# awslabs/crowd-coachable-recommendations

Hardware: AMD Instinct MI355X
Metric: queries/sec, exhaustive inner-product top-100 retrieval (NQ-shaped 2,681,468 x 768 bf16 corpus) (higher is better)
Workload: dtype bf16

## Files before the change

### crowd-coachable-recommendations_amd/ccrec_amd/_lib.py

```python
import ctypes
import os

_HERE = os.path.dirname(os.path.abspath(__file__))
LIB_PATH = os.path.join(os.path.dirname(_HERE), "lib", "libccr_hip.so")

CCR_OK = 0
CCR_ERR_INVALID, CCR_ERR_HIP, CCR_ERR_WORKSPACE, CCR_ERR_BLOCK_ID = -1, -2, -3, -4
DTYPE_F32, DTYPE_F16, DTYPE_BF16 = 0, 1, 2
SEARCH_DEFAULT, SEARCH_FORCE_DENSE, SEARCH_FORCE_FUSED, SEARCH_ASYNC = 0, 1, 2, 4
SCORES_CANONICAL, SCORES_MFMA = 0, 1

EXPORTS = [
    "ccr_last_error", "ccr_version", "ccr_pack_bf16", "ccr_pack_bf16_ex", "ccr_meanpool_pack_bf16", "ccr_meanpool_pack_bf16_ex", "ccr_index_create",
    "ccr_index_create_with_norms", "ccr_index_destroy",
    "ccr_index_rows", "ccr_index_dim", "ccr_search_workspace_bytes", "ccr_search", "ccr_search_last_stats",
    "ccr_merge_topk", "ccr_merge_topk_strided", "ccr_apply_block", "ccr_inbatch_ce_workspace_bytes", "ccr_inbatch_ce_fwd", "ccr_inbatch_ce_bwd", "ccr_inbatch_ce_bwd_dev", "ccr_rank_metrics",
    "ccr_search_finish", "ccr_scores", "ccr_search_blocked_workspace_bytes", "ccr_search_blocked",
    "ccr_search_sparse_prior_workspace_bytes", "ccr_search_sparse_prior", "ccr_colsum_bf16", "ccr_meanpool_bwd", "ccr_bm25_index_create", "ccr_bm25_index_destroy", "ccr_bm25_search_workspace_bytes",
    "ccr_bm25_search", "ccr_pack_bf16_padded", "ccr_shard_message_bytes", "ccr_search_shard", "ccr_shard_message_fill", "ccr_merge_shard_messages",
    "ccr_attention_bf16", "ccr_add_layernorm", "ccr_meanpool_pack_bf16_packed", "ccr_embed_layernorm", "ccr_gelu_bf16",
    "ccr_attention_half", "ccr_add_layernorm_half", "ccr_embed_layernorm_half", "ccr_gelu_half", "ccr_merge_short_lists",
    "ccr_bm25_search_workspace_bytes_k", "ccr_bm25_search_last_stats", "ccr_bm25_index_set_idf", "ccr_inbatch_pack3_bf16", "ccr_inbatch_ce_fwd_f32",
    "ccr_search_stream_wait_main_pass", "ccr_pool_ce_workspace_bytes", "ccr_pool_ce_fwd", "ccr_pool_ce_fwd_f32", "ccr_pool_ce_bwd_dev",
    "ccr_bpr_sample", "ccr_bpr_frozen_workspace_bytes", "ccr_bpr_frozen_fwd", "ccr_bpr_frozen_bwd_dev",
    "ccr_attention_fwd_train_half", "ccr_attention_bwd_workspace_bytes", "ccr_attention_bwd_half", "ccr_add_layernorm_bwd_half", "ccr_gelu_bwd_half",
    "ccr_dropout_bits_rows", "ccr_dropout_bits_attention", "ccr_dropout_apply", "ccr_attention_fwd_train_drop_half", "ccr_attention_bwd_drop_half",
    "ccr_add_layernorm_drop_half", "ccr_add_layernorm_bwd_drop_half", "ccr_search_last_main_split",
    "ccr_search_last_threshold_phases", "ccr_adamw_step",
    "ccr_embed_layernorm_train_half", "ccr_embed_layernorm_bwd_half", "ccr_embedding_grad", "ccr_meanpool_bwd_packed",
    "ccr_pack_half_ex", "ccr_pack_half_padded", "ccr_meanpool_pack_half_ex", "ccr_meanpool_pack_half_packed", "ccr_index_create_half",
    "ccr_index_create_with_norms_half", "ccr_index_dtype", "ccr_colsum_half",
    "ccr_grad_stats_workspace_bytes", "ccr_grad_stats", "ccr_adamw_control_update", "ccr_adamw_step_scaled",
    "ccr_keep_f32", "ccr_rescore_f32_workspace_bytes", "ccr_rescore_f32",
    "ccr_attention_bias_half",
]

MIN_VERSION = 101
BPR_VERSION = 102
ENCODER_TRAIN_VERSION = 103
ENCODER_DROPOUT_VERSION = 104
QSPLIT_VERSION = 105
THR_PHASES_VERSION = 106
OPTIM_VERSION = 107
ENCODER_PACKED_TRAIN_VERSION = 108
HALF_INDEX_VERSION = 109
AMP_OPTIM_VERSION = 110
RANK_F32_VERSION = 111
ATTENTION_BIAS_VERSION = 112

SHARD_HEADER_BYTES = 32
SHARD_MAGIC = 0x4D524343


class ShardHeader(ctypes.Structure):
    _fields_ = [("magic", ctypes.c_uint32), ("n_flagged", ctypes.c_uint32), ("k_valid", ctypes.c_uint32),
                ("n_covered", ctypes.c_uint32), ("row_offset", ctypes.c_int64), ("n_rows", ctypes.c_int64)]


class SearchStats(ctypes.Structure):
    _fields_ = [("path", ctypes.c_int32), ("n_fallback", ctypes.c_int32), ("sample_tiles", ctypes.c_int32),
                ("ranges", ctypes.c_int32), ("cap", ctypes.c_int32), ("sublists", ctypes.c_int32),
                ("n_candidates", ctypes.c_int64), ("ms_sample", ctypes.c_float), ("ms_threshold", ctypes.c_float),
                ("ms_main", ctypes.c_float), ("ms_select", ctypes.c_float), ("ms_fallback", ctypes.c_float),
                ("ms_total", ctypes.c_float), ("n_retried", ctypes.c_int32), ("n_dense", ctypes.c_int32),
                ("main_launches", ctypes.c_int32), ("opt_rank", ctypes.c_int32), ("main_tile_queries", ctypes.c_int32),
                ("skipped_tiles", ctypes.c_int32), ("tile_cap", ctypes.c_int32)]


class AdamwSegment(ctypes.Structure):
    _fields_ = [("param", ctypes.c_void_p), ("grad", ctypes.c_void_p), ("exp_avg", ctypes.c_void_p), ("exp_avg_sq", ctypes.c_void_p),
                ("shadow", ctypes.c_void_p), ("n", ctypes.c_int64), ("decay", ctypes.c_float), ("step_size", ctypes.c_float),
                ("bc2_sqrt", ctypes.c_float), ("shadow_dtype", ctypes.c_int32)]


class AdamwControl(ctypes.Structure):
    _fields_ = [("coef", ctypes.c_float), ("skip", ctypes.c_int32), ("norm", ctypes.c_float), ("scale", ctypes.c_float),
                ("growth_tracker", ctypes.c_int32), ("skipped_total", ctypes.c_int32), ("reserved", ctypes.c_uint32 * 10)]


CONTROL_WORDS = {name: i for i, (name, _) in enumerate(AdamwControl._fields_[:6])}


class CcrError(RuntimeError):
    pass


_lib = None


def load():
    global _lib
    if _lib is not None:
        return _lib
    if not os.path.isfile(LIB_PATH):
        raise CcrError(f"{LIB_PATH} not built: run `python -c 'import __graft_entry__ as g; g.build()'` "
                       f"(or make -C crowd-coachable-recommendations_amd/csrc)")
    lib = ctypes.CDLL(LIB_PATH)
    lib.ccr_version.restype = ctypes.c_int
    have = int(lib.ccr_version())
    if have < MIN_VERSION:
        raise CcrError(f"{LIB_PATH} is version {have}, this binding needs {MIN_VERSION}: rebuild it "
                       f"(python -c 'import __graft_entry__ as g; g.build()')")
    missing = [name for name in EXPORTS if not hasattr(lib, name)]
    if missing:
        raise CcrError(f"{LIB_PATH} lacks {', '.join(missing)}: rebuild it (python -c 'import __graft_entry__ as g; g.build()')")
    vp, i32, i64, f32, sz = ctypes.c_void_p, ctypes.c_int, ctypes.c_int64, ctypes.c_float, ctypes.c_size_t
    lib.ccr_last_error.restype = ctypes.c_char_p
    lib.ccr_last_error.argtypes = []
    lib.ccr_version.restype = i32
    lib.ccr_pack_bf16.argtypes = [vp, vp, vp, i64, i32, i32, vp]
    lib.ccr_pack_bf16_ex.argtypes = [vp, vp, vp, vp, i64, i32, i32, vp]
    lib.ccr_index_create_with_norms.argtypes = [vp, i64, i32, i64, vp, vp, ctypes.POINTER(vp)]
    lib.ccr_meanpool_pack_bf16.argtypes = [vp, i32, vp, vp, vp, i32, i32, i32, i32, vp]
    lib.ccr_meanpool_pack_bf16_ex.argtypes = [vp, i32, vp, vp, vp, vp, vp, i32, i32, i32, i32, vp]
    lib.ccr_index_create.argtypes = [vp, i64, i32, i64, vp, ctypes.POINTER(vp)]
    lib.ccr_index_destroy.argtypes = [vp]
    lib.ccr_index_rows.argtypes = [vp]
    lib.ccr_index_rows.restype = i64
    lib.ccr_index_dim.argtypes = [vp]
    lib.ccr_search_workspace_bytes.argtypes = [vp, i32, i32]
    lib.ccr_search_workspace_bytes.restype = sz
    lib.ccr_search.argtypes = [vp, vp, i32, i32, vp, vp, vp, sz, i32, vp]
    lib.ccr_search_last_stats.argtypes = [vp, ctypes.POINTER(SearchStats)]
    lib.ccr_merge_topk.argtypes = [vp, vp, i32, i32, i32, vp, vp, vp]
    lib.ccr_merge_topk_strided.argtypes = [vp, vp, i64, i64, i32, i32, i32, vp, vp, vp]
    lib.ccr_apply_block.argtypes = [vp, vp, i32, i32, vp, vp, i64, vp, vp, i32, vp]
    lib.ccr_inbatch_ce_workspace_bytes.argtypes = [i32, i32]
    lib.ccr_inbatch_ce_workspace_bytes.restype = sz
    lib.ccr_inbatch_ce_fwd.argtypes = [vp, vp, vp, i32, i32, f32, vp, vp, vp, sz, vp]
    lib.ccr_inbatch_ce_bwd.argtypes = [vp, vp, vp, vp, i32, i32, f32, f32, vp, vp, vp, vp, sz, vp]
    lib.ccr_inbatch_ce_bwd_dev.argtypes = [vp, vp, vp, vp, i32, i32, f32, vp, vp, vp, vp, vp, sz, vp]
    lib.ccr_inbatch_pack3_bf16.argtypes = [vp, vp, vp, i32, i32, vp, vp]
    lib.ccr_inbatch_ce_fwd_f32.argtypes = [vp, vp, vp, i32, i32, f32, vp, vp, vp, vp, sz, vp]
    lib.ccr_pool_ce_workspace_bytes.argtypes = [i32, i32, i32]
    lib.ccr_pool_ce_workspace_bytes.restype = sz
    lib.ccr_pool_ce_fwd.argtypes = [vp, vp, vp, vp, i32, i32, i32, f32, vp, vp, vp, sz, vp]
    lib.ccr_pool_ce_fwd_f32.argtypes = [vp, vp, vp, vp, i32, i32, i32, f32, vp, vp, vp, vp, sz, vp]
    lib.ccr_pool_ce_bwd_dev.argtypes = [vp, vp, vp, vp, vp, i32, i32, i32, f32, vp, vp, vp, vp, vp, sz, vp]
    lib.ccr_bpr_sample.argtypes = [vp, i32, i32, i64, vp, vp, vp, f32, vp, vp, i32, vp, i32, vp, vp]
    lib.ccr_bpr_frozen_workspace_bytes.argtypes = [i32, i32, i32]
    lib.ccr_bpr_frozen_workspace_bytes.restype = sz
    lib.ccr_bpr_frozen_fwd.argtypes = [vp, i64, i32, vp, vp, f32, vp, vp, vp, vp, i32, i32, vp, vp, sz, vp]
    lib.ccr_bpr_frozen_bwd_dev.argtypes = [vp, i64, i32, vp, vp, f32, vp, vp, vp, vp, i32, i32, vp, vp, vp, vp, vp, sz, vp]
    lib.ccr_rank_metrics.argtypes = [vp, i32, i32, vp, vp, vp, i32, vp, vp, vp]
    lib.ccr_search_finish.argtypes = [vp]
    lib.ccr_search_stream_wait_main_pass.argtypes = [vp, vp]
    lib.ccr_search_last_main_split.argtypes = [vp]
    lib.ccr_search_last_threshold_phases.argtypes = [vp]
    lib.ccr_scores.argtypes = [vp, vp, i32, i32, vp, vp]
    lib.ccr_search_blocked_workspace_bytes.argtypes = [vp, i32, i32, vp]
    lib.ccr_search_blocked_workspace_bytes.restype = sz
    lib.ccr_search_blocked.argtypes = [vp, vp, i32, i32, vp, vp, vp, vp, vp, sz, i32, vp]
    lib.ccr_search_sparse_prior_workspace_bytes.argtypes = [vp, i32, i32, vp]
    lib.ccr_search_sparse_prior_workspace_bytes.restype = sz
    lib.ccr_search_sparse_prior.argtypes = [vp, vp, i32, i32, vp, vp, vp, vp, vp, vp, sz, i32, vp]
    lib.ccr_colsum_bf16.argtypes = [vp, i64, i32, vp, vp]
    lib.ccr_meanpool_bwd.argtypes = [vp, vp, vp, i32, i32, i32, i32, vp]
    lib.ccr_bm25_index_create.argtypes = [vp, vp, vp, vp, i64, i64, ctypes.c_double, ctypes.POINTER(vp)]
    lib.ccr_bm25_index_destroy.argtypes = [vp]
    lib.ccr_bm25_search_workspace_bytes.argtypes = [vp, i32, i32]
    lib.ccr_bm25_search_workspace_bytes.restype = sz
    lib.ccr_bm25_search_workspace_bytes_k.argtypes = [vp, i32, i32, i32]
    lib.ccr_bm25_search_workspace_bytes_k.restype = sz
    lib.ccr_bm25_search_last_stats.argtypes = [vp, vp]
    lib.ccr_bm25_index_set_idf.argtypes = [vp, vp, vp, vp]
    lib.ccr_bm25_search.argtypes = [vp, vp, vp, vp, i32, i32, vp, vp, vp, sz, vp]
    lib.ccr_pack_bf16_padded.argtypes = [vp, i64, i32, vp, i32, vp, vp, i32, vp]
    lib.ccr_attention_bf16.argtypes = [vp, vp, vp, vp, i32, i32, i32, i32, ctypes.c_float, vp]
    lib.ccr_add_layernorm.argtypes = [vp, vp, vp, vp, ctypes.c_float, vp, vp, i64, i32, vp]
    lib.ccr_embed_layernorm.argtypes = [vp, i64, vp, i64, vp, i64, vp, vp, vp, vp, vp, ctypes.c_float, vp, vp, i64, i32, vp]
    lib.ccr_gelu_bf16.argtypes = [vp, vp, i64, vp]
    lib.ccr_attention_half.argtypes = [vp, vp, vp, vp, i32, i32, i32, i32, ctypes.c_float, i32, vp]
    lib.ccr_attention_bias_half.argtypes = [vp, vp, vp, vp, vp, i32, i32, i32, i32, i32, ctypes.c_float, i32, vp]
    lib.ccr_add_layernorm_half.argtypes = [vp, vp, vp, vp, ctypes.c_float, vp, vp, i64, i32, i32, vp]
    lib.ccr_embed_layernorm_half.argtypes = [vp, i64, vp, i64, vp, i64, vp, vp, vp, vp, vp, ctypes.c_float, vp, vp, i64, i32, i32, vp]
    lib.ccr_gelu_half.argtypes = [vp, vp, i64, i32, vp]
    lib.ccr_attention_fwd_train_half.argtypes = [vp, vp, vp, vp, vp, i32, i32, i32, i32, ctypes.c_float, i32, vp]
    lib.ccr_attention_bwd_workspace_bytes.argtypes = [i32, i32, i32]
    lib.ccr_attention_bwd_workspace_bytes.restype = sz
    lib.ccr_attention_bwd_half.argtypes = [vp, vp, vp, vp, vp, vp, vp, i32, i32, i32, i32, ctypes.c_float, i32, vp, sz, vp]
    lib.ccr_add_layernorm_bwd_half.argtypes = [vp, vp, vp, ctypes.c_float, vp, vp, vp, vp, vp, i64, i32, i32, vp, sz, vp]
    lib.ccr_gelu_bwd_half.argtypes = [vp, vp, vp, i64, i32, vp]
    u64, u32, f64 = ctypes.c_uint64, ctypes.c_uint32, ctypes.c_double
    lib.ccr_dropout_bits_rows.argtypes = [vp, i64, i32, u64, u32, f64, vp]
    lib.ccr_dropout_bits_attention.argtypes = [vp, vp, vp, vp, i64, i32, i32, i32, u64, u32, f64, vp]
    lib.ccr_dropout_apply.argtypes = [vp, vp, f32, vp, vp, i64, i32, i32, vp]
    lib.ccr_attention_fwd_train_drop_half.argtypes = [vp, vp, vp, vp, vp, vp, f32, i32, i32, i32, i32, f32, i32, vp]
    lib.ccr_attention_bwd_drop_half.argtypes = [vp, vp, vp, vp, vp, vp, vp, vp, f32, vp, i32, i32, i32, i32, f32, i32, vp, sz, vp]
    lib.ccr_add_layernorm_drop_half.argtypes = [vp, vp, f32, vp, vp, vp, f32, vp, vp, i64, i32, i32, vp]
    lib.ccr_add_layernorm_bwd_drop_half.argtypes = [vp, vp, f32, vp, vp, f32, vp, vp, vp, vp, vp, i64, i32, i32, vp, sz, vp]
    lib.ccr_adamw_step.argtypes = [vp, i32, f32, f32, f32, f32, vp]
    lib.ccr_grad_stats_workspace_bytes.argtypes = [vp, i32]
    lib.ccr_grad_stats_workspace_bytes.restype = i64
    lib.ccr_grad_stats.argtypes = [vp, i32, vp, vp]
    lib.ccr_adamw_control_update.argtypes = [vp, vp, i64, f32, i32, ctypes.c_double, ctypes.c_double, i32, vp, vp, vp]
    lib.ccr_adamw_step_scaled.argtypes = [vp, i32, f32, f32, f32, f32, vp, vp]
    lib.ccr_embed_layernorm_train_half.argtypes = [vp, i64, vp, i64, vp, i64, vp, vp, vp, vp, vp, f32, vp, f32, vp, vp, i64, i32, i32, vp]
    lib.ccr_embed_layernorm_bwd_half.argtypes = [vp, i64, vp, i64, vp, i64, vp, vp, vp, vp, f32, vp, f32, vp, vp, vp, vp, i64, i32, vp, sz, vp]
    lib.ccr_embedding_grad.argtypes = [vp, vp, vp, i64, i32, vp, i64, vp]
    lib.ccr_meanpool_bwd_packed.argtypes = [vp, vp, vp, vp, i32, i32, i32, vp]
    lib.ccr_meanpool_pack_bf16_packed.argtypes = [vp, i32, vp, vp, vp, vp, vp, vp, i32, i32, i32, vp]
    lib.ccr_pack_half_ex.argtypes = [vp, vp, vp, vp, i64, i32, i32, i32, vp, vp]
    lib.ccr_pack_half_padded.argtypes = [vp, i64, i32, vp, i32, vp, vp, i32, i32, vp, vp]
    lib.ccr_meanpool_pack_half_ex.argtypes = [vp, i32, vp, vp, vp, vp, vp, i32, i32, i32, i32, i32, vp, vp]
    lib.ccr_meanpool_pack_half_packed.argtypes = [vp, i32, vp, vp, vp, vp, vp, vp, i32, i32, i32, i32, vp, vp]
    lib.ccr_index_create_half.argtypes = [vp, i64, i32, i32, i64, vp, ctypes.POINTER(vp)]
    lib.ccr_index_create_with_norms_half.argtypes = [vp, i64, i32, i32, i64, vp, vp, ctypes.POINTER(vp)]
    lib.ccr_index_dtype.argtypes = [vp]
    lib.ccr_colsum_half.argtypes = [vp, i64, i32, i32, vp, vp]
    lib.ccr_keep_f32.argtypes = [vp, vp, i32, i32, vp, vp, i64, i32, vp]
    lib.ccr_rescore_f32_workspace_bytes.argtypes = [i32, i32, i32, i32]
    lib.ccr_rescore_f32_workspace_bytes.restype = sz
    lib.ccr_rescore_f32.argtypes = [vp, vp, i64, i32, vp, vp, i32, i32, i32, i64, vp, vp, vp, vp, vp, vp, vp, sz, vp]
    lib.ccr_shard_message_bytes.argtypes = [i32, i32]
    lib.ccr_shard_message_bytes.restype = sz
    lib.ccr_search_shard.argtypes = [vp, vp, i32, i32, vp, vp, sz, i32, vp]
    lib.ccr_shard_message_fill.argtypes = [vp, i32, i32, i32, vp, vp, i64, i64, vp]
    lib.ccr_merge_shard_messages.argtypes = [vp, i64, i32, i32, i32, vp, vp, vp]
    lib.ccr_merge_short_lists.argtypes = [vp, i64, i32, i32, i32, i32, vp, vp, vp, vp, vp]
    for name in EXPORTS:
        fn = getattr(lib, name)
        if fn.restype is ctypes.c_int and name not in ("ccr_version", "ccr_index_dim", "ccr_index_dtype"):
            fn.restype = i32
    _lib = lib
    return lib


def check(rc, what=""):
    if rc != CCR_OK:
        msg = load().ccr_last_error().decode("utf-8", "replace")
        if rc == CCR_ERR_BLOCK_ID:
            raise AssertionError("block id not found")
        raise CcrError(f"{what} failed ({rc}): {msg}")
```

### crowd-coachable-recommendations_amd/csrc/ccr_api.hip

```cpp
#include <stdarg.h>
#include <stdlib.h>
#include <string.h>

#include <math.h>

#include <algorithm>
#include <mutex>
#include <set>
#include <utility>
#include <vector>

#include "ccr_index.h"
#include "ccr_narrow.h"
#include "ccr_topk_device.h"

namespace ccr {

static thread_local char g_err[512] = "";
void set_error(const char *fmt, ...) {
    va_list ap;
    va_start(ap, fmt);
    vsnprintf(g_err, sizeof(g_err), fmt, ap);
    va_end(ap);
}

}

using namespace ccr;

namespace {
constexpr int SLAB_SLOTS = 1024, SLAB_SLOT_BYTES = 256, MAX_DEVICES = 64;
struct Slab {
    char *base = nullptr;
    char *host = nullptr;
    std::vector<int> free_slots;
};
constexpr int SLAB_HOST_BYTES = 64;
std::mutex g_slab_mutex;
Slab g_slabs[MAX_DEVICES];

int slab_take(int device, uint32_t **out, volatile uint32_t **host_out) {
    std::lock_guard<std::mutex> lock(g_slab_mutex);
    CCR_REQUIRE(device >= 0 && device < MAX_DEVICES, "device ordinal %d out of range", device);
    Slab &sl = g_slabs[device];
    if (!sl.base) {
        CCR_HIP_CHECK(hipMalloc((void **)&sl.base, (size_t)SLAB_SLOTS * SLAB_SLOT_BYTES));
        if (hipHostMalloc((void **)&sl.host, (size_t)SLAB_SLOTS * SLAB_HOST_BYTES, hipHostMallocDefault) != hipSuccess) {
            (void)hipFree(sl.base);
            sl.base = nullptr;
            set_error("ccr_index_create: hipHostMalloc of the pinned flag lines failed");
            return CCR_ERR_HIP;
        }
        for (int i = SLAB_SLOTS - 1; i >= 0; --i) sl.free_slots.push_back(i);
    }
    if (sl.free_slots.empty()) {
        set_error("ccr_index_create: more than %d live indices on device %d", SLAB_SLOTS, device);
        return CCR_ERR_INVALID;
    }
    *out = reinterpret_cast<uint32_t *>(sl.base + (size_t)sl.free_slots.back() * SLAB_SLOT_BYTES);
    *host_out = reinterpret_cast<volatile uint32_t *>(sl.host + (size_t)sl.free_slots.back() * SLAB_HOST_BYTES);
    sl.free_slots.pop_back();
    return CCR_OK;
}

void slab_give(int device, uint32_t *p) {
    if (!p || device < 0 || device >= MAX_DEVICES) return;
    std::lock_guard<std::mutex> lock(g_slab_mutex);
    Slab &sl = g_slabs[device];
    sl.free_slots.push_back((int)((reinterpret_cast<char *>(p) - sl.base) / SLAB_SLOT_BYTES));
}
}

extern "C" const char *ccr_last_error(void) { return g_err; }
extern "C" int ccr_version(void) { return 112; }

extern "C" int ccr_index_destroy(ccr_index *ix);

namespace {
struct CachedBlock {
    void *p;
    size_t bytes;
};
std::vector<CachedBlock> g_blocks[MAX_DEVICES];
constexpr size_t BLOCK_CACHE_ENTRIES = 8;

int block_take(int device, size_t bytes, void **out, size_t *got) {
    CCR_REQUIRE(device >= 0 && device < MAX_DEVICES, "device ordinal %d out of range", device);
    bytes = (bytes + 4095) / 4096 * 4096;
    {
        std::lock_guard<std::mutex> lock(g_slab_mutex);
        auto &v = g_blocks[device];
        for (size_t i = 0; i < v.size(); ++i)
            if (v[i].bytes >= bytes && v[i].bytes <= 2 * bytes) {
                *out = v[i].p;
                *got = v[i].bytes;
                v.erase(v.begin() + i);
                return CCR_OK;
            }
    }
    CCR_HIP_CHECK(hipMalloc(out, bytes));
    *got = bytes;
    return CCR_OK;
}

void block_give(int device, void *p, size_t bytes) {
    if (!p) return;
    void *drop = nullptr;
    if (device >= 0 && device < MAX_DEVICES && bytes <= ((size_t)64 << 20)) {
        std::lock_guard<std::mutex> lock(g_slab_mutex);
        auto &v = g_blocks[device];
        v.push_back({p, bytes});
        if (v.size() > BLOCK_CACHE_ENTRIES) {
            drop = v.front().p;
            v.erase(v.begin());
        }
    } else {
        drop = p;
    }
    if (drop) (void)hipFree(drop);
}
}

int ccr::ensure_dynamic_lds(const void *kernel, size_t lds) {
    static std::mutex mu;
    static std::set<std::pair<const void *, int>> done;
    int dev = 0;
    CCR_HIP_CHECK(hipGetDevice(&dev));
    std::lock_guard<std::mutex> lock(mu);
    if (done.count({kernel, dev})) return CCR_OK;
    CCR_HIP_CHECK(hipFuncSetAttribute(kernel, hipFuncAttributeMaxDynamicSharedMemorySize, (int)lds));
    done.insert({kernel, dev});
    return CCR_OK;
}

static int index_create_impl(const uint16_t *D_bf16, int half_dtype, int64_t n_rows, int dim, int64_t global_row_offset, const float *row_bounds,
                             void *stream, ccr_index **out) {
    CCR_REQUIRE(D_bf16 && out, "ccr_index_create: null pointer");
    if (const int rc = check_half("ccr_index_create", half_dtype)) return rc;
    CCR_REQUIRE(n_rows >= 1 && n_rows < ((int64_t)1 << 32), "ccr_index_create: n_rows=%lld out of range [1, 2^32)",
                (long long)n_rows);
    CCR_REQUIRE(dim >= 8 && dim % 8 == 0 && dim <= 4096, "ccr_index_create: dim=%d must be a multiple of 8 in [8, 4096]", dim);
    CCR_REQUIRE((uintptr_t)D_bf16 % 16 == 0, "ccr_index_create: corpus pointer must be 16-byte aligned");
    hipStream_t s = (hipStream_t)stream;
    ccr_index *ix = new ccr_index();
    memset(ix, 0, sizeof(*ix));
    ix->D = D_bf16;
    ix->dtype = half_dtype;
    ix->n_rows = n_rows;
    ix->dim = dim;
    ix->offset = ix->id_out = global_row_offset;
    ix->knobs = read_knobs();
    auto build = [&]() -> int {
        CCR_HIP_CHECK(hipGetDevice(&ix->device));
        CCR_HIP_CHECK(hipDeviceGetAttribute(&ix->num_cu, hipDeviceAttributeMultiprocessorCount, ix->device));
        int rc = slab_take(ix->device, &ix->dmax_bits, &ix->host_flags);
        if (rc != CCR_OK) return rc;
        const int64_t tiles = (n_rows + TILE_DOCS - 1) / TILE_DOCS;
        void *tn = nullptr;
        rc = block_take(ix->device, (size_t)tiles * 4, &tn, &ix->tile_bytes);
        if (rc != CCR_OK) return rc;
        ix->tile_norm = (float *)tn;
        uint32_t *tile_bits = reinterpret_cast<uint32_t *>(ix->tile_norm);
        if (row_bounds) {
            ix->row_norm = row_bounds;
            rc = launch_tile_norms(row_bounds, n_rows, tile_bits, ix->dmax_bits, s);
            if (rc != CCR_OK) return rc;
        } else {
            void *rn = nullptr;
            rc = block_take(ix->device, (size_t)n_rows * 4, &rn, &ix->row_bytes);
            if (rc != CCR_OK) return rc;
            ix->row_norm = ix->row_norm_own = (float *)rn;
            CCR_HIP_CHECK(hipMemsetAsync(ix->dmax_bits, 0, 4, s));
            CCR_HIP_CHECK(hipMemsetAsync(tile_bits, 0, (size_t)tiles * 4, s));
            rc = launch_row_norms(D_bf16, half_dtype, n_rows, dim, ix->row_norm_own, ix->dmax_bits, tile_bits, s);
            if (rc != CCR_OK) return rc;
            CCR_HIP_CHECK(hipStreamSynchronize(s));
        }
        return CCR_OK;
    };
    const int rc = build();
    if (rc != CCR_OK) {
        ccr_index_destroy(ix);
        return rc;
    }
    *out = ix;
    return CCR_OK;
}

extern "C" int ccr_index_create_half(const uint16_t *D, int64_t n_rows, int dim, int half_dtype, int64_t global_row_offset, void *stream,
                                     ccr_index **out) {
    return index_create_impl(D, half_dtype, n_rows, dim, global_row_offset, nullptr, stream, out);
}

extern "C" int ccr_index_create_with_norms_half(const uint16_t *D, int64_t n_rows, int dim, int half_dtype, int64_t global_row_offset,
                                                const float *row_norm_bounds, void *stream, ccr_index **out) {
    CCR_REQUIRE(row_norm_bounds, "ccr_index_create_with_norms: null row_norm_bounds");
    return index_create_impl(D, half_dtype, n_rows, dim, global_row_offset, row_norm_bounds, stream, out);
}

extern "C" int ccr_index_create(const uint16_t *D_bf16, int64_t n_rows, int dim, int64_t global_row_offset, void *stream,
                                ccr_index **out) {
    return ccr_index_create_half(D_bf16, n_rows, dim, CCR_DTYPE_BF16, global_row_offset, stream, out);
}

extern "C" int ccr_index_create_with_norms(const uint16_t *D_bf16, int64_t n_rows, int dim, int64_t global_row_offset,
                                           const float *row_norm_bounds, void *stream, ccr_index **out) {
    return ccr_index_create_with_norms_half(D_bf16, n_rows, dim, CCR_DTYPE_BF16, global_row_offset, row_norm_bounds, stream, out);
}

extern "C" int ccr_index_destroy(ccr_index *ix) {
    if (!ix) return CCR_OK;
    if (ix->pending.active && ix->have_events) (void)hipEventSynchronize(ix->ev[EV_ASYNC_END]);
    ix->pending.active = false;
    slab_give(ix->device, ix->dmax_bits);
    block_give(ix->device, ix->tile_norm, ix->tile_bytes);
    block_give(ix->device, ix->row_norm_own, ix->row_bytes);
    if (ix->have_events)
        for (int i = 0; i < EV_COUNT; ++i)
            if (ix->ev[i]) (void)hipEventDestroy(ix->ev[i]);
    delete ix;
    return CCR_OK;
}

extern "C" int64_t ccr_index_rows(const ccr_index *ix) { return ix ? ix->n_rows : -1; }
extern "C" int ccr_index_dim(const ccr_index *ix) { return ix ? ix->dim : -1; }
extern "C" int ccr_index_dtype(const ccr_index *ix) { return ix ? ix->dtype : -1; }

extern "C" size_t ccr_search_workspace_bytes(const ccr_index *ix, int n_q, int k) {
    if (!ix || n_q <= 0 || k <= 0) return 0;
    Plan a = make_plan(ix->n_rows, ix->dim, n_q, k, CCR_SEARCH_DEFAULT, ix->num_cu, ix->knobs);
    Plan b = make_plan(ix->n_rows, ix->dim, n_q, k, CCR_SEARCH_FORCE_DENSE, ix->num_cu, ix->knobs);
    Plan c = make_plan(ix->n_rows, ix->dim, n_q, k, CCR_SEARCH_FORCE_FUSED, ix->num_cu, ix->knobs);
    return std::max({a.total, b.total, c.total}) + 256;
}

extern "C" int ccr_search_stream_wait_main_pass(const ccr_index *ix, void *stream) {
    CCR_REQUIRE(ix, "ccr_search_stream_wait_main_pass: null index");
    if (!ix->main_pass_recorded) return CCR_OK;
    CCR_HIP_CHECK(hipStreamWaitEvent((hipStream_t)stream, ix->ev[EV_MAIN_END], 0));
    return CCR_OK;
}

extern "C" int ccr_search_last_stats(const ccr_index *ix, ccr_search_stats *stats) {
    CCR_REQUIRE(ix && stats, "ccr_search_last_stats: null pointer");
    CCR_REQUIRE(!ix->pending.active, "ccr_search_last_stats: an asynchronous search is pending (call ccr_search_finish first)");
    *stats = ix->stats;
    return CCR_OK;
}

extern "C" int ccr_search_last_main_split(const ccr_index *ix) {
    if (!ix || ix->plan_nq <= 0 || !ix->plan.fused) return 0;
    return ix->plan.main_qsplit;
}

extern "C" int ccr_search_last_threshold_phases(const ccr_index *ix) {
    if (!ix || ix->plan_nq <= 0 || !ix->plan.fused) return 0;
    return ix->thr_phases_used;
}

static int dense_for_list(const ccr_index *ix, const uint16_t *Q, const uint32_t *d_qlist, int n, int k, float *scratch, int64_t rows_per_chunk,
                          float *out_scores, int64_t *out_ids, hipStream_t s) {
    for (int lo = 0; lo < n; lo += (int)rows_per_chunk) {
        const int m = std::min<int64_t>(rows_per_chunk, n - lo);
        int rc = launch_dense_scores(ix->D, ix->dtype, ix->n_rows, ix->dim, Q, d_qlist ? d_qlist + lo : nullptr, lo, m, nullptr, scratch, s);
        if (rc != CCR_OK) return rc;
        rc = launch_dense_select(scratch, ix->n_rows, k, d_qlist ? d_qlist + lo : nullptr, lo, m, nullptr, ix->id_out, out_scores, out_ids, s);
        if (rc != CCR_OK) return rc;
    }
    return CCR_OK;
}

static bool margin_path_ok(const ccr_index *ix, int k) { return ix->dim % 8 == 0 && k <= MAX_K; }
static int64_t tiles_of(const ccr_index *ix) { return (ix->n_rows + TILE_DOCS - 1) / TILE_DOCS; }

static GemmArgs gemm_args(const ccr_index *ix, const uint16_t *Q, int n_q, int nq_pad) {
    GemmArgs g;
    memset(&g, 0, sizeof(g));
    g.D = ix->D;
    g.n_rows = ix->n_rows;
    g.dim = ix->dim;
    g.Q = Q;
    g.n_q = n_q;
    g.nq_pad = nq_pad;
    g.qblocks = nq_pad / TILE_Q;
    g.item_end = INT32_MAX;
    return g;
}

static GemmArgs filter_args(const ccr_index *ix, const Plan &p, const SearchWs &w, const uint16_t *Q, int n_q, int nq_pad, int qblocks,
                            int qgroups, const float *thr, const float *cq, const CandLayout &lay) {
    GemmArgs g = gemm_args(ix, Q, n_q, nq_pad);
    g.qblocks = qblocks;
    g.qgroups = qgroups;
    g.n_vt = p.tiles;
    g.tile_stride = 1;
    g.ranges = p.ranges;
    g.thr = thr;
    g.cq = cq;
    g.tile_norm = ix->tile_norm;
    g.cnt = w.cnt;
    g.cand = w.cand;
    g.lay = lay;
    return g;
}

static ThresholdArgs threshold_args(const ccr_index *ix, const SearchWs &w) {
    const Plan &p = ix->plan;
    ThresholdArgs t{};
    t.gmax = w.gmax, t.n_groups = (int64_t)p.sample_tiles * GROUPS_PER_TILE, t.sample_stride = p.sample_stride;
    t.n_q = ix->pending.n_q, t.nq_pad = p.nq_pad, t.k = ix->pending.k, t.qnorm = w.qnorm;
    t.dmax_bits = ix->dmax_bits, t.dim = ix->dim, t.tile_norm = ix->tile_norm;
    t.thr = w.thr, t.cq = w.cq, t.phases = ix->knobs.thr_phases;
    return t;
}

static ThresholdUpdateArgs update_args(const ccr_index *ix, const SearchWs &w) {
    ThresholdUpdateArgs u{};
    u.cand = w.cand, u.cnt = w.cnt, u.sp = ix->plan.sublists;
    u.n_q = ix->pending.n_q, u.nq_pad = ix->plan.nq_pad, u.k = ix->pending.k;
    u.cq = w.cq, u.tile_norm = ix->tile_norm, u.thr = w.thr;
    return u;
}

static SelectArgs select_args(const ccr_index *ix, const SearchWs &w) {
    const Plan &p = ix->plan;
    const auto &pd = ix->pending;
    SelectArgs a{};
    a.cand = w.cand, a.cnt = w.cnt, a.n_q = pd.n_q, a.nq_pad = p.nq_pad;
    a.k = pd.k, a.rescore_cap = p.rescore_cap, a.regular_cap = p.rescore_regular, a.compact = p.select_compact;
    a.D = ix->D, a.dt = ix->dtype, a.dim = ix->dim, a.n_rows = ix->n_rows;
    a.tile_norm = ix->tile_norm, a.row_norm = ix->row_norm, a.dmax_bits = ix->dmax_bits, a.id_offset = ix->id_out;
    a.Q = pd.Q, a.thr = w.thr, a.cq = w.cq;
    a.out_scores = pd.out_scores, a.out_ids = pd.out_ids;
    return a;
}

static int store_scores(const ccr_index *ix, const uint16_t *Q, int n_q, int ranges, float *out, int64_t pitch, hipStream_t s) {
    GemmArgs g = gemm_args(ix, Q, n_q, (int)round_up(n_q, TILE_Q));
    g.n_vt = tiles_of(ix);
    g.tile_stride = 1;
    g.ranges = ranges;
    g.qgroups = 1;
    g.store = out;
    g.store_pitch = pitch;
    return launch_gemm(g, ix->dtype, ix->knobs.mfma16 != 0 ? MAIN_16X16 : MAIN_32X32, EPI_STORE, std::max(NUM_XCD, ix->num_cu / NUM_XCD * NUM_XCD), s);
}

static int margin_for_rows(const ccr_index *ix, const uint16_t *Qc, const float *hint, const uint32_t *out_rows, int n, int k, float *scratch,
                           size_t scratch_bytes, float *out_scores, int64_t *out_ids, uint32_t *flag_count, uint32_t *flag_list, hipStream_t s) {
    const int64_t pitch = round_up(ix->n_rows, 4);
    int64_t chunk = (int64_t)(scratch_bytes / ((size_t)pitch * 4));
    CCR_REQUIRE(chunk >= 1, "margin path: no room for one score row");
    if (chunk > TILE_Q) chunk = chunk / TILE_Q * TILE_Q;
    const int ranges = (int)round_up(std::min<int64_t>(std::max<int64_t>(1, tiles_of(ix) / 4), 1024), NUM_XCD);
    for (int lo = 0; lo < n; lo += (int)chunk) {
        const int m = std::min<int64_t>(chunk, n - lo);
        const uint16_t *Q = Qc + (int64_t)lo * ix->dim;
        int rc = store_scores(ix, Q, m, ranges, scratch, pitch, s);
        if (rc != CCR_OK) return rc;
        rc = launch_margin_select(scratch, pitch, ix->n_rows, k, ix->dim, Q, ix->D, ix->dtype, ix->tile_norm, ix->row_norm, ix->dmax_bits,
                                  hint ? hint + lo : nullptr, out_rows ? out_rows + lo : nullptr, lo, m, ix->id_out, out_scores, out_ids, flag_count, flag_list, s);
        if (rc != CCR_OK) return rc;
    }
    return CCR_OK;
}

static int run_main_pass(const ccr_index *ix, const Plan &p, const SearchWs &w, const uint16_t *Q, int n_q, hipStream_t s) {
    GemmArgs gm = filter_args(ix, p, w, Q, n_q, p.nq_pad, p.main_qblocks, p.main_qgroups, w.thr, w.cq, p.cand);
    gm.qsplit = p.main_qsplit;
    if (p.skip_sampled) {
        gm.n_vt = p.tiles - p.sample_tiles;
        gm.skip_stride = (int)p.sample_stride;
        gm.skip_count = p.sample_tiles;
    }
    const int nrc = NUM_XCD / gm.qgroups, qb_per = gm.qblocks / gm.qgroups, items = p.ranges / nrc * qb_per;
    const int bounds[4] = {0, p.item_a, p.item_b, items};
    ThresholdUpdateArgs u = update_args(ix, w);
    u.lay = p.cand, u.qb_per = qb_per, u.tile_q = p.tile_q, u.top = p.item_b ? w.top : nullptr;
    int done = 0;
    for (int ph = 1; ph < 4; ++ph) {
        if (bounds[ph] <= done) continue;
        if (done > 0) {
            const int rl_full = done / qb_per;
            u.part_blocks = done % qb_per;
            u.nsub = rl_full * nrc * p.sublists;
            u.nsub_part = u.part_blocks ? (rl_full + 1) * nrc * p.sublists : 0;
            u.top_out = bounds[ph] < items && ph < 3;
            const int rc = launch_threshold_update(u, s);
            if (rc != CCR_OK) return rc;
            u.prev_nsub = u.nsub, u.prev_part = u.nsub_part, u.prev_blocks = u.part_blocks, u.top_in = true;
        }
        gm.item_begin = done;
        gm.item_end = bounds[ph];
        const MainKernel kind = p.tile_q == WIDE_Q ? MAIN_WIDE : p.mfma16 ? MAIN_16X16 : MAIN_32X32;
        const int rc = launch_gemm(gm, ix->dtype, kind, EPI_FILTER, p.grid, s);
        if (rc != CCR_OK) return rc;
        done = bounds[ph];
    }
    return CCR_OK;
}

static int run_narrow_pass(const ccr_index *ix, const Plan &p, const SearchWs &w, const uint16_t *Q, int n_q, hipStream_t s) {
    NarrowArgs na;
    memset(&na, 0, sizeof(na));
    na.D = ix->D;
    na.n_rows = ix->n_rows;
    na.dim = ix->dim;
    na.Q = Q;
    na.n_q = n_q;
    na.q_stride = narrow_query_stride(ix->dim);
    na.thr = w.thr;
    na.cq = w.cq;
    na.tile_norm = ix->tile_norm;
    na.cand = w.cand;
    na.cnt = w.cnt;
    na.cap = p.first_lay.cap[0];
    na.groups = p.narrow_groups;
    int ngrid = ix->knobs.narrow_grid > 0 ? ix->knobs.narrow_grid : ix->num_cu;
    const int64_t blocks = (ix->n_rows + 16 * NARROW_WAVES - 1) / (16 * NARROW_WAVES);
    if ((int64_t)ngrid > blocks) ngrid = (int)std::max<int64_t>(1, blocks);
    if (p.narrow_groups == 2) ngrid = std::max(16, ngrid / 16 * 16);
    return launch_narrow_filter(na, ix->dtype, p.narrow, ngrid, s);
}

static int read_words(void *host, const void *dev, int n, hipStream_t s) {
    CCR_HIP_CHECK(hipMemcpyAsync(host, dev, (size_t)n * 4, hipMemcpyDeviceToHost, s));
    CCR_HIP_CHECK(hipStreamSynchronize(s));
    return CCR_OK;
}


static int fused_stats(ccr_index *ix, uint32_t nflag, unsigned long long ncand) {
    const Plan &p = ix->plan;
    ccr_search_stats &st = ix->stats;
    float a = 0, b = 0;
    CCR_HIP_CHECK(hipEventElapsedTime(&st.ms_sample, ix->ev[EV_SAMPLE_BEGIN], ix->ev[EV_SAMPLE_END]));
    CCR_HIP_CHECK(hipEventElapsedTime(&a, ix->ev[EV_BEGIN], ix->ev[EV_SAMPLE_BEGIN]));
    CCR_HIP_CHECK(hipEventElapsedTime(&b, ix->ev[EV_SAMPLE_END], ix->ev[EV_MAIN_BEGIN]));
    st.ms_threshold = a + b;
    CCR_HIP_CHECK(hipEventElapsedTime(&st.ms_main, ix->ev[EV_MAIN_BEGIN], ix->ev[EV_MAIN_END]));
    CCR_HIP_CHECK(hipEventElapsedTime(&st.ms_select, ix->ev[EV_MAIN_END], ix->ev[EV_SELECT_END]));
    CCR_HIP_CHECK(hipEventElapsedTime(&st.ms_total, ix->ev[EV_BEGIN], ix->ev[EV_SELECT_END]));
    st.path = 1;
    st.n_fallback = (int32_t)nflag;
    st.sample_tiles = p.sample_tiles;
    st.ranges = p.narrow ? 1 : p.ranges;
    st.cap = p.narrow ? p.first_lay.cap[0] : p.cap;
    st.sublists = p.narrow ? p.first_sp : p.sublists;
    st.main_launches = 1 + (p.item_a ? 1 : 0) + (p.item_b ? 1 : 0);
    st.opt_rank = p.opt_rank;
    st.tile_cap = p.opt_rank ? p.tile_cap : 0;
    st.skipped_tiles = p.skip_sampled ? p.sample_tiles : 0;
    st.main_tile_queries = p.narrow ? 0 : p.tile_q;
    st.n_candidates = (int64_t)ncand;
    return CCR_OK;
}

static int recover_thresholds(const ccr_index *ix, const SearchWs &w, int nflag) {
    hipStream_t s = ix->pending.stream;
    ThresholdArgs t = threshold_args(ix, w);
    t.thr = w.thr_safe, t.cq = w.cq_safe;
    const int rc = launch_threshold(t, s);
    if (rc != CCR_OK) return rc;
    return launch_underfilled_to_retry(w.flag_list, 0, nflag, w.thr_safe, w.thr, s);
}

static int to_dense(const SearchWs &w, const uint32_t *list, int n, int &n_dense, hipStream_t s) {
    CCR_HIP_CHECK(hipMemcpyAsync(w.dense_list + n_dense, list, (size_t)n * 4, hipMemcpyDeviceToDevice, s));
    n_dense += n;
    return CCR_OK;
}

static int retry_group(ccr_index *ix, const SearchWs &w, const uint32_t *cur, int n_cur, int &n_dense) {
    const Plan &p = ix->plan;
    const auto &pd = ix->pending;
    hipStream_t s = pd.stream;
    const int nsub_all = p.ranges * p.sublists;
    for (int round = 0;; ++round) {
        int rc = launch_gather_queries(pd.Q, ix->dim, cur, n_cur, w.thr, w.cq, w.Q2, w.thr2, w.cq2, s);
        if (rc != CCR_OK) return rc;
        const int pad2 = (int)round_up(n_cur, TILE_Q);
        const int64_t cap2 = std::min<int64_t>(8192, (int64_t)(w.cand_bytes / 8) / ((int64_t)nsub_all * pad2) / 4 * 4);
        if (cap2 < 16) break;
        const CandLayout lay2 = one_segment((int)cap2);
        CCR_HIP_CHECK(hipMemsetAsync(w.cnt, 0, (size_t)nsub_all * pad2 * 4, s));
        CCR_HIP_CHECK(hipMemsetAsync(w.flag2, 0, 64, s));
        const GemmArgs g = filter_args(ix, p, w, w.Q2, n_cur, pad2, pad2 / TILE_Q, pick_qgroups(pad2 / TILE_Q, ix->dim, ix->knobs), w.thr2, w.cq2, lay2);
        rc = launch_gemm(g, ix->dtype, p.mfma16 ? MAIN_16X16 : MAIN_32X32, EPI_FILTER, p.grid, s);
        if (rc != CCR_OK) return rc;
        SelectArgs sel = select_args(ix, w);
        sel.ranges = nsub_all, sel.sp = p.sublists, sel.lay = lay2, sel.n_q = n_cur, sel.nq_pad = pad2;
        sel.Q = w.Q2, sel.thr = w.thr2, sel.cq = w.cq2, sel.out_rows = cur;
        sel.flag_count = w.flag2, sel.flag_list = w.flag2 + 16;
        rc = launch_select_rescore(sel, s);
        if (rc != CCR_OK) return rc;
        ix->stats.n_retried += n_cur;
        uint32_t again = 0;
        rc = read_words(&again, w.flag2, 1, s);
        if (rc != CCR_OK || again == 0) return rc;
        uint32_t *next = (cur == w.list_b) ? w.list_c : w.list_b;
        rc = launch_partition_flags(w.flag2 + 16, 0, (int)again, next, w.dense_list + n_dense, w.counts, s);
        if (rc != CCR_OK) return rc;
        uint32_t hc[2] = {0, 0};
        rc = read_words(hc, w.counts, 2, s);
        if (rc != CCR_OK) return rc;
        n_dense += (int)hc[1];
        const uint32_t *list = cur;
        const int n = n_cur;
        cur = next;
        n_cur = (int)hc[0];
        if (n_cur == 0 || round == 2 || n_cur >= n) break;
        ThresholdUpdateArgs u = update_args(ix, w);
        u.nsub = nsub_all, u.lay = lay2, u.n_q = n, u.nq_pad = pad2, u.cq = w.cq2, u.thr = w.thr2;
        rc = launch_threshold_update(u, s);
        if (rc != CCR_OK) return rc;
        rc = launch_scatter_thresholds(list, n, w.thr2, w.thr, s);
        if (rc != CCR_OK) return rc;
    }
    return n_cur > 0 ? to_dense(w, cur, n_cur, n_dense, s) : CCR_OK;
}

static int retry_flagged(ccr_index *ix, const SearchWs &w, int n_retry, int &n_dense) {
    const Plan &p = ix->plan;
    const auto &pd = ix->pending;
    const int nsub_all = p.ranges * p.sublists;
    if (nsub_all > 2048) return to_dense(w, w.retry_list, n_retry, n_dense, pd.stream);
    ThresholdUpdateArgs u = update_args(ix, w);
    u.nsub = p.first_nsub, u.sp = p.first_sp, u.lay = p.first_lay;
    int rc = launch_threshold_update(u, pd.stream);
    if (rc != CCR_OK) return rc;
    const int64_t want_cap = std::min<int64_t>(8192, 4 * (int64_t)p.cap);
    int64_t group = (int64_t)(w.cand_bytes / 8) / ((int64_t)nsub_all * want_cap) / TILE_Q * TILE_Q;
    group = std::max<int64_t>(TILE_Q, std::min<int64_t>(group, round_up(n_retry, TILE_Q)));
    for (int g0 = 0; g0 < n_retry && rc == CCR_OK; g0 += (int)group)
        rc = retry_group(ix, w, w.retry_list + g0, std::min<int>((int)group, n_retry - g0), n_dense);
    return rc;
}

static int complete_dense(ccr_index *ix, const SearchWs &w, int n_dense) {
    const Plan &p = ix->plan;
    const auto &pd = ix->pending;
    hipStream_t s = pd.stream;
    const bool margin_in_cand = w.cand_bytes > w.dense_bytes;
    const int64_t fit = (int64_t)(w.cand_bytes / ((size_t)ix->n_rows * 4)) / 64 * 64;
    const bool fp64_in_cand = n_dense > p.dense_rows_per_chunk && fit >= 64;
    const int64_t chunk = fp64_in_cand ? std::min<int64_t>(fit, 256) : p.dense_rows_per_chunk;
    float *fp64_scr = fp64_in_cand ? (float *)w.cand : w.dense;
    if (!margin_path_ok(ix, pd.k))
        return dense_for_list(ix, pd.Q, w.dense_list, n_dense, pd.k, fp64_scr, chunk, pd.out_scores, pd.out_ids, s);
    CCR_HIP_CHECK(hipMemsetAsync(w.flag2, 0, 64, s));
    for (int lo = 0; lo < n_dense; lo += p.nq_pad) {
        const int m = std::min(p.nq_pad, n_dense - lo);
        int rc = launch_gather_queries(pd.Q, ix->dim, w.dense_list + lo, m, w.thr, w.cq, w.Q2, w.thr2, w.cq2, s);
        if (rc != CCR_OK) return rc;
        rc = margin_for_rows(ix, w.Q2, w.thr2, w.dense_list + lo, m, pd.k, margin_in_cand ? (float *)w.cand : w.dense,
                             margin_in_cand ? w.cand_bytes : w.dense_bytes, pd.out_scores, pd.out_ids, w.flag2, w.flag2 + 16, s);
        if (rc != CCR_OK) return rc;
    }
    uint32_t left = 0;
    const int rc = read_words(&left, w.flag2, 1, s);
    if (rc != CCR_OK || left == 0) return rc;
    return dense_for_list(ix, pd.Q, w.flag2 + 16, (int)left, pd.k, fp64_scr, chunk, pd.out_scores, pd.out_ids, s);
}

static int search_complete(ccr_index *ix) {
    auto &pd = ix->pending;
    hipStream_t s = pd.stream;
    const bool was_async = pd.active;
    pd.active = false;
    const SearchWs w = search_ws(ix->plan, ix->n_rows, ix->dim, pd.n_q, pd.k, pd.ws);
    struct { uint32_t nflag, pad; unsigned long long ncand; } host;
    int rc = CCR_OK;
    if (was_async) {
        CCR_HIP_CHECK(hipEventSynchronize(ix->ev[EV_ASYNC_END]));
        host.nflag = ix->host_flags[0];
        host.ncand = *reinterpret_cast<volatile unsigned long long *>(ix->host_flags + 2);
    } else {
        rc = read_words(&host, w.flag_count, 4, s);
        if (rc != CCR_OK) return rc;
    }
    rc = fused_stats(ix, host.nflag, host.ncand);
    if (rc != CCR_OK || host.nflag == 0) return rc;
    rc = ix->plan.opt_rank ? recover_thresholds(ix, w, (int)host.nflag) : CCR_OK;
    if (rc != CCR_OK) return rc;
    rc = launch_partition_flags(w.flag_list, 0, (int)host.nflag, w.retry_list, w.dense_list, w.counts, s);
    if (rc != CCR_OK) return rc;
    uint32_t hc[2] = {0, 0};
    rc = read_words(hc, w.counts, 2, s);
    if (rc != CCR_OK) return rc;
    int n_dense = (int)hc[1];
    if (hc[0] > 0) rc = retry_flagged(ix, w, (int)hc[0], n_dense);
    if (rc == CCR_OK && n_dense > 0) rc = complete_dense(ix, w, n_dense);
    if (rc != CCR_OK) return rc;
    ix->stats.n_dense += n_dense;
    CCR_HIP_CHECK(hipEventRecord(ix->ev[EV_DONE], s));
    CCR_HIP_CHECK(hipStreamSynchronize(s));
    CCR_HIP_CHECK(hipEventElapsedTime(&ix->stats.ms_fallback, ix->ev[EV_SELECT_END], ix->ev[EV_DONE]));
    ix->stats.ms_total += ix->stats.ms_fallback;
    return CCR_OK;
}

extern "C" int ccr_search_finish(ccr_index *ix) {
    CCR_REQUIRE(ix, "ccr_search_finish: null index");
    return ix->pending.active ? search_complete(ix) : CCR_OK;
}

static int search_dense(ccr_index *ix, const SearchWs &w, const uint16_t *Q, int n_q, int k, float *out_scores, int64_t *out_ids,
                        int flags, hipStream_t s) {
    const bool async = (flags & CCR_SEARCH_ASYNC) != 0;
    const int64_t chunk = ix->plan.dense_rows_per_chunk;
    int rc;
    if (!async && !(flags & CCR_SEARCH_FORCE_DENSE) && margin_path_ok(ix, k)) {
        CCR_HIP_CHECK(hipMemsetAsync(w.flag_count, 0, 64, s));
        rc = margin_for_rows(ix, Q, nullptr, nullptr, n_q, k, w.dense, w.dense_bytes, out_scores, out_ids, w.flag_count, w.flag_list, s);
        if (rc != CCR_OK) return rc;
        uint32_t nf = 0;
        rc = read_words(&nf, w.flag_count, 1, s);
        if (rc != CCR_OK) return rc;
        ix->stats.n_fallback = ix->stats.n_dense = (int32_t)nf;
        if (nf > 0) rc = dense_for_list(ix, Q, w.flag_list, (int)nf, k, w.dense, chunk, out_scores, out_ids, s);
    } else {
        rc = dense_for_list(ix, Q, nullptr, n_q, k, w.dense, chunk, out_scores, out_ids, s);
    }
    if (rc != CCR_OK) return rc;
    CCR_HIP_CHECK(hipEventRecord(ix->ev[EV_DONE], s));
    if (async) return CCR_OK;
    CCR_HIP_CHECK(hipStreamSynchronize(s));
    CCR_HIP_CHECK(hipEventElapsedTime(&ix->stats.ms_total, ix->ev[EV_BEGIN], ix->ev[EV_DONE]));
    ix->stats.ms_fallback = ix->stats.ms_total;
    return CCR_OK;
}

static int search_impl(ccr_index *ix, const uint16_t *Q_bf16, int n_q, int k, float *out_scores, int64_t *out_ids, int64_t id_out,
                       uint32_t *flagged_out, void *workspace, size_t ws_bytes, int flags, void *stream) {
    CCR_REQUIRE(ix && Q_bf16 && out_scores && out_ids, "ccr_search: null pointer");
    CCR_REQUIRE(n_q >= 0, "ccr_search: n_q=%d", n_q);
    CCR_REQUIRE(k >= 1 && k <= MAX_K && (int64_t)k <= ix->n_rows, "ccr_search: k=%d must be in [1, min(n_rows=%lld, %d)]", k,
                (long long)ix->n_rows, MAX_K);
    CCR_REQUIRE((uintptr_t)Q_bf16 % 16 == 0, "ccr_search: query pointer must be 16-byte aligned");
    CCR_REQUIRE(!ix->pending.active, "ccr_search: an asynchronous search is pending on this index (call ccr_search_finish first)");
    memset(&ix->stats, 0, sizeof(ix->stats));
    ix->main_pass_recorded = false;
    ix->thr_phases_used = 0;
    if (n_q == 0) return CCR_OK;
    hipStream_t s = (hipStream_t)stream;
    ix->id_out = id_out;
    const bool async = (flags & CCR_SEARCH_ASYNC) != 0;
    const int plan_flags = flags & ~CCR_SEARCH_ASYNC;
    if (!(ix->plan_nq == n_q && ix->plan_k == k && ix->plan_flags == plan_flags)) {
        ix->plan = make_plan(ix->n_rows, ix->dim, n_q, k, plan_flags, ix->num_cu, ix->knobs);
        ix->plan_nq = n_q;
        ix->plan_k = k;
        ix->plan_flags = plan_flags;
    }
    const Plan p = ix->plan;
    if (!workspace || ws_bytes < p.total || (uintptr_t)workspace % 256 != 0) {
        set_error("ccr_search: workspace %zu bytes (256-byte aligned) required, got %zu at %p", p.total, ws_bytes, workspace);
        return CCR_ERR_WORKSPACE;
    }
    const SearchWs w = search_ws(p, ix->n_rows, ix->dim, n_q, k, (char *)workspace);

    if (!ix->have_events) {
        for (int i = 0; i < EV_COUNT; ++i) CCR_HIP_CHECK(hipEventCreate(&ix->ev[i]));
        ix->have_events = true;
    }
    CCR_HIP_CHECK(hipEventRecord(ix->ev[EV_BEGIN], s));
    if (!p.fused) return search_dense(ix, w, Q_bf16, n_q, k, out_scores, out_ids, flags, s);
    ix->pending = {false, Q_bf16, n_q, k, out_scores, out_ids, (char *)workspace, s};

    CCR_HIP_CHECK(hipMemsetAsync(w.flag_count, 0, 64, s));
    if ((int64_t)p.ranges > p.tiles - (p.skip_sampled ? p.sample_tiles : 0)) CCR_HIP_CHECK(hipMemsetAsync(w.cnt, 0, (size_t)p.ranges * p.nq_pad * p.sublists * 4, s));
    int rc = launch_row_norms(Q_bf16, ix->dtype, n_q, ix->dim, w.qnorm, nullptr, nullptr, s);
    if (rc != CCR_OK) return rc;

    GemmArgs gs = gemm_args(ix, Q_bf16, n_q, p.nq_pad);
    gs.qgroups = p.qgroups;
    gs.n_vt = p.sample_tiles;
    gs.tile_stride = p.sample_stride;
    gs.ranges = p.sample_ranges;
    gs.gmax = w.gmax;
    CCR_HIP_CHECK(hipEventRecord(ix->ev[EV_SAMPLE_BEGIN], s));
    rc = launch_gemm(gs, ix->dtype, MAIN_32X32, EPI_GMAX, p.grid, s);
    if (rc != CCR_OK) return rc;
    CCR_HIP_CHECK(hipEventRecord(ix->ev[EV_SAMPLE_END], s));
    const bool skip_list = p.skip_sampled && ix->knobs.skip_list;
    ThresholdArgs t = threshold_args(ix, w);
    if (p.opt_rank) t.k = p.opt_rank, t.tile_cap = p.tile_cap;
    if (p.narrow) t.zero_cnt = w.cnt, t.zero_per_query = NARROW_SUBLISTS;
    if (skip_list) t.glist = w.glist, t.list_cap = skip_list_cap(p.opt_rank);
    rc = launch_threshold(t, s, &ix->thr_phases_used);
    if (rc != CCR_OK) return rc;

    CCR_HIP_CHECK(hipEventRecord(ix->ev[EV_MAIN_BEGIN], s));
    rc = p.narrow ? run_narrow_pass(ix, p, w, Q_bf16, n_q, s) : run_main_pass(ix, p, w, Q_bf16, n_q, s);
    if (rc != CCR_OK) return rc;
    CCR_HIP_CHECK(hipEventRecord(ix->ev[EV_MAIN_END], s));
    ix->main_pass_recorded = true;
    SelectArgs sel = select_args(ix, w);
    sel.ranges = p.first_nsub, sel.sp = p.first_sp, sel.lay = p.first_lay;
    sel.flag_count = w.flag_count, sel.flag_list = w.flag_list, sel.stat_cand = w.stat_cand;
    if (p.skip_sampled)
        sel.gmax = w.gmax, sel.sample_tiles = p.sample_tiles, sel.sample_stride = (int)p.sample_stride, sel.gmax_pitch = p.nq_pad;
    if (skip_list) sel.glist = w.glist, sel.list_cap = t.list_cap;
    rc = launch_select_rescore(sel, s);
    if (rc != CCR_OK) return rc;
    CCR_HIP_CHECK(hipEventRecord(ix->ev[EV_SELECT_END], s));

    if (!async) return search_complete(ix);
    if (flagged_out) CCR_HIP_CHECK(hipMemcpyAsync(flagged_out, w.flag_count, 4, hipMemcpyDeviceToDevice, s));
    CCR_HIP_CHECK(hipMemcpyAsync((void *)ix->host_flags, w.flag_count, 16, hipMemcpyDeviceToHost, s));
    CCR_HIP_CHECK(hipEventRecord(ix->ev[EV_ASYNC_END], s));
    ix->pending.active = true;
    return CCR_OK;
}

extern "C" int ccr_search(ccr_index *ix, const uint16_t *Q_bf16, int n_q, int k, float *out_scores, int64_t *out_ids,
                          void *workspace, size_t ws_bytes, int flags, void *stream) {
    CCR_REQUIRE(ix, "ccr_search: null index");
    return search_impl(ix, Q_bf16, n_q, k, out_scores, out_ids, ix->offset, nullptr, workspace, ws_bytes, flags, stream);
}

static inline size_t shard_rows_at(int n_q, int k) { return (sizeof(ccr_shard_header) + (size_t)n_q * k * 4 + 15) / 16 * 16; }

extern "C" size_t ccr_shard_message_bytes(int n_q, int k) {
    if (n_q < 0 || k < 1) return 0;
    return (shard_rows_at(n_q, k) + (size_t)n_q * k * 4 + 15) / 16 * 16;
}

extern "C" int ccr_search_shard(ccr_index *ix, const uint16_t *Q_bf16, int n_q, int k, void *message, void *workspace, size_t ws_bytes,
                                int flags, void *stream) {
    CCR_REQUIRE(ix && message, "ccr_search_shard: null pointer");
    CCR_REQUIRE((uintptr_t)message % 16 == 0, "ccr_search_shard: message must be 16-byte aligned");
    CCR_REQUIRE(n_q >= 0 && k >= 1, "ccr_search_shard: bad shape n_q=%d k=%d", n_q, k);
    hipStream_t s = (hipStream_t)stream;
    ccr_shard_header h;
    memset(&h, 0, sizeof(h));
    h.magic = CCR_SHARD_MAGIC;
    h.k_valid = (uint32_t)k;
    h.n_covered = 0u;
    h.row_offset = ix->offset;
    h.n_rows = ix->n_rows;
    int rc = launch_shard_header(h, message, s);
    if (rc != CCR_OK) return rc;
    if (n_q == 0) return CCR_OK;
    char *m = (char *)message;
    uint32_t *flagged = reinterpret_cast<uint32_t *>(m + offsetof(ccr_shard_header, n_flagged));
    return search_impl(ix, Q_bf16, n_q, k, reinterpret_cast<float *>(m + sizeof(ccr_shard_header)),
                       reinterpret_cast<int64_t *>(m + shard_rows_at(n_q, k)), ID_LOCAL_U32, flagged, workspace, ws_bytes, flags, stream);
}

extern "C" int ccr_scores(const ccr_index *ix, const uint16_t *Q_bf16, int n_q, int mode, float *out, void *stream) {
    CCR_REQUIRE(ix && Q_bf16 && out && n_q > 0, "ccr_scores: bad argument");
    CCR_REQUIRE((uintptr_t)Q_bf16 % 16 == 0, "ccr_scores: query pointer must be 16-byte aligned");
    if (mode == CCR_SCORES_CANONICAL)
        return launch_dense_scores(ix->D, ix->dtype, ix->n_rows, ix->dim, Q_bf16, nullptr, 0, n_q, nullptr, out, (hipStream_t)stream);
    CCR_REQUIRE(mode == CCR_SCORES_MFMA, "ccr_scores: unknown mode %d", mode);
    CCR_REQUIRE(ix->dim % 8 == 0, "ccr_scores: CCR_SCORES_MFMA needs dim %% 8 == 0 (dim=%d)", ix->dim);
    return store_scores(ix, Q_bf16, n_q, (int)round_up(std::min<int64_t>(64, tiles_of(ix)), NUM_XCD), out, 0, (hipStream_t)stream);
}
```

### crowd-coachable-recommendations_amd/csrc/ccr_common.h

```cpp
#pragma once
#include <hip/hip_runtime.h>
#include <stdint.h>
#include <stdio.h>

#include <type_traits>

#include "ccr_retrieval.h"

namespace ccr {

void set_error(const char *fmt, ...);

#define CCR_HIP_CHECK(expr)                                                                   \
    do {                                                                                      \
        hipError_t _e = (expr);                                                               \
        if (_e != hipSuccess) {                                                               \
            ccr::set_error("%s failed: %s (%s:%d)", #expr, hipGetErrorString(_e), __FILE__, __LINE__); \
            return CCR_ERR_HIP;                                                               \
        }                                                                                     \
    } while (0)

#define CCR_REQUIRE(cond, ...)            \
    do {                                  \
        if (!(cond)) {                    \
            ccr::set_error(__VA_ARGS__);  \
            return CCR_ERR_INVALID;       \
        }                                 \
    } while (0)

#define CCR_LAUNCH_CHECK()                                                              \
    do {                                                                                \
        hipError_t _e = hipGetLastError();                                              \
        if (_e != hipSuccess) {                                                         \
            ccr::set_error("kernel launch failed: %s (%s:%d)", hipGetErrorString(_e), __FILE__, __LINE__); \
            return CCR_ERR_HIP;                                                         \
        }                                                                               \
    } while (0)

constexpr int TILE_DOCS = 256;
constexpr int TILE_Q = 256;
constexpr int WIDE_Q = 384;
constexpr int TILE_K = 32;
constexpr int GEMM_THREADS = 512;
constexpr int GROUPS_PER_TILE = 16;
constexpr int MAX_K = 4096;
constexpr uint32_t FLAG_DENSE = 0x80000000u;
constexpr int NUM_XCD = 8;

struct CandLayout {
    int nseg;
    int seg_end[3];
    int cap[3];
    long long base[3];
};
__host__ __device__ __forceinline__ void cand_segment(const CandLayout &L, int r, int &cap, int &r0, long long &base) {
    const int g = (r >= L.seg_end[0] ? 1 : 0) + (r >= L.seg_end[1] ? 1 : 0);
    r0 = g ? L.seg_end[g - 1] : 0;
    cap = L.cap[g];
    base = L.base[g];
}
__host__ __device__ __forceinline__ long long cand_sublist(const CandLayout &L, int r, int q, int s, int nq_pad, int sp, int &cap) {
    const int g = (r >= L.seg_end[0] ? 1 : 0) + (r >= L.seg_end[1] ? 1 : 0);
    const int r0 = g ? L.seg_end[g - 1] : 0;
    cap = L.cap[g];
    return L.base[g] + (((long long)(r - r0) * nq_pad + q) * sp) * (long long)cap + s;
}

__host__ __device__ __forceinline__ int64_t unsampled_tile(int64_t v, int s, int n) {
    if (s == 0) return v;
    const uint32_t u = (uint32_t)v, d = (uint32_t)(s - 1);
    return u < (uint32_t)n * d ? (int64_t)(u + u / d + 1u) : v + n;
}

__host__ __device__ __forceinline__ int64_t main_item(int i, int xcd, int qblocks, int qgroups, int qsplit, int ranges, int64_t n_vt, int &r,
                                                      int &qb) {
    const int groups = qsplit ? qsplit : qgroups, g = xcd % groups, rc = xcd / groups, nrc = NUM_XCD / groups;
    const int base = qblocks / groups;
    int rl, b;
    if (qsplit == 0) {
        rl = i / base;
        b = g * base + i % base;
    } else {
        const int rem = qblocks - base * groups;
        const int period = i / qblocks, o = i - period * qblocks;
        int row = g, k = o - g * base;
        if (k < 0) {
            row = o / base;
            k = o - row * base;
        } else if (k >= base + rem) {
            row = (o - rem) / base;
            k = o - rem - row * base;
        }
        rl = period * groups + row;
        b = k >= base ? groups * base + (k - base) : g * base + k;
    }
    const int ri = rc + nrc * rl;
    const int64_t ntile = (n_vt - ri + ranges - 1) / ranges;
    r = ri;
    qb = b;
    return ntile;
}

enum { EPI_FILTER = 0, EPI_GMAX = 1, EPI_STORE = 2 };

struct GemmArgs {
    const uint16_t *D;
    int64_t n_rows;
    int dim;
    const uint16_t *Q;
    int n_q;
    int nq_pad;
    int qblocks;
    int64_t n_vt;
    int64_t tile_stride;
    int ranges;
    int skip_stride, skip_count;
    int qgroups;
    int qsplit;
    int item_begin, item_end;
    const float *thr;
    const float *cq;
    const float *tile_norm;
    uint2 *cand;
    uint32_t *cnt;
    CandLayout lay;
    float *gmax;
    float *store;
    int64_t store_pitch;
};


template <class F>
inline int dispatch_half(int half_dtype, F &&f) {
    return half_dtype == CCR_DTYPE_F16 ? f(std::integral_constant<int, CCR_DTYPE_F16>{}) : f(std::integral_constant<int, CCR_DTYPE_BF16>{});
}
inline int check_half(const char *who, int half_dtype) {
    CCR_REQUIRE(half_dtype == CCR_DTYPE_BF16 || half_dtype == CCR_DTYPE_F16, "%s: half_dtype=%d (CCR_DTYPE_F16 or CCR_DTYPE_BF16)", who, half_dtype);
    return CCR_OK;
}

template <int DT>
__device__ __forceinline__ float elem_to_f32(uint16_t h) {
    if constexpr (DT == CCR_DTYPE_F16)
        return (float)__builtin_bit_cast(_Float16, h);
    else
        return __uint_as_float(((uint32_t)h) << 16);
}
template <int DT>
__device__ __forceinline__ float elem_lo(uint32_t w) {
    if constexpr (DT == CCR_DTYPE_F16)
        return elem_to_f32<DT>((uint16_t)w);
    else
        return __uint_as_float(w << 16);
}
template <int DT>
__device__ __forceinline__ float elem_hi(uint32_t w) {
    if constexpr (DT == CCR_DTYPE_F16)
        return elem_to_f32<DT>((uint16_t)(w >> 16));
    else
        return __uint_as_float(w & 0xffff0000u);
}

__device__ __forceinline__ double wave_sumsq(const float *__restrict__ x, int dim, int lane) {
    double p = 0.0;
    const int nchunk = dim >> 2;
    for (int c = lane; c < nchunk; c += 64) {
        float4 v = reinterpret_cast<const float4 *>(x)[c];
        p = p + (double)v.x * (double)v.x;
        p = p + (double)v.y * (double)v.y;
        p = p + (double)v.z * (double)v.z;
        p = p + (double)v.w * (double)v.w;
    }
#pragma unroll
    for (int off = 32; off >= 1; off >>= 1) p = p + __shfl_xor(p, off, 64);
    return p;
}

__device__ __forceinline__ uint32_t f32_orderable(float f) {
    uint32_t u = __float_as_uint(f);
    return (u & 0x80000000u) ? ~u : (u | 0x80000000u);
}
__device__ __forceinline__ float orderable_to_f32(uint32_t u) {
    return __uint_as_float((u & 0x80000000u) ? (u & 0x7fffffffu) : ~u);
}

constexpr int64_t ID_LOCAL_U32 = INT64_MIN;
__device__ __forceinline__ void store_id(int64_t *out_ids, int64_t pos, int64_t id_offset, uint32_t row) {
    if (id_offset == ID_LOCAL_U32)
        reinterpret_cast<uint32_t *>(out_ids)[pos] = row;
    else
        out_ids[pos] = id_offset + (int64_t)row;
}

__host__ __device__ __forceinline__ float mfma_gamma(int dim) { return (float)dim * 1.1920929e-7f * 1.02f; }

}
```

### crowd-coachable-recommendations_amd/csrc/ccr_index.h

```cpp
#pragma once
#include "ccr_common.h"
#include "ccr_plan.h"

namespace ccr {

enum MainKernel { MAIN_32X32, MAIN_16X16, MAIN_WIDE };
int launch_gemm(const GemmArgs &a, int dt, MainKernel kind, int epi, int grid, hipStream_t s);
int launch_shard_header(const ccr_shard_header &h, void *message, hipStream_t s);
int ensure_dynamic_lds(const void *kernel, size_t lds);
int launch_row_norms(const uint16_t *X, int dt, int64_t rows, int dim, float *norms, uint32_t *max_bits, uint32_t *tile_bits,
                     hipStream_t s);
int launch_tile_norms(const float *row_bounds, int64_t rows, uint32_t *tile_bits, uint32_t *max_bits, hipStream_t s);

struct ThresholdArgs {
    const float *gmax;
    int64_t n_groups, sample_stride;
    int n_q, nq_pad, dim;
    int k;
    int tile_cap = GROUPS_PER_TILE;
    const float *qnorm, *tile_norm;
    const uint32_t *dmax_bits;
    float *thr, *cq;
    uint32_t *zero_cnt = nullptr; int zero_per_query = 0;
    uint32_t *glist = nullptr; int list_cap = 0;
    int phases = 0;
};
int launch_threshold(const ThresholdArgs &a, hipStream_t s, int *phases_used = nullptr);

struct ThresholdUpdateArgs {
    const uint2 *cand;
    const uint32_t *cnt;
    CandLayout lay;
    int sp;
    int n_q, nq_pad, k, nsub;
    const float *cq, *tile_norm;
    float *thr;
    int nsub_part = 0, part_blocks = 0, prev_nsub = 0, prev_part = 0, prev_blocks = 0;
    int qb_per = 1;
    uint32_t *top = nullptr;
    bool top_in = false, top_out = false;
    int tile_q = TILE_Q;
};
int launch_threshold_update(const ThresholdUpdateArgs &a, hipStream_t s);

int select_compact_entries(int dim, int ranges, int rescore_cap, int64_t want);
struct SelectArgs {
    const uint2 *cand;
    const uint32_t *cnt;
    CandLayout lay;
    int ranges, sp, n_q, nq_pad;
    int k, rescore_cap, compact;
    int regular_cap;
    const uint16_t *D;
    int dt, dim;
    int64_t n_rows, id_offset;
    const float *tile_norm, *row_norm;
    const uint32_t *dmax_bits;
    const uint16_t *Q;
    float *thr;
    const float *cq;
    float *out_scores;
    int64_t *out_ids;
    const uint32_t *out_rows = nullptr;
    uint32_t *flag_count, *flag_list;
    unsigned long long *stat_cand = nullptr;
    const float *gmax = nullptr; int sample_tiles = 0, sample_stride = 0, gmax_pitch = 0;
    const uint32_t *glist = nullptr; int list_cap = 0;
};
int launch_select_rescore(const SelectArgs &a, hipStream_t s);
int launch_partition_flags(const uint32_t *flags, int begin, int n, uint32_t *retry_list, uint32_t *dense_list, uint32_t *counts,
                           hipStream_t s);
int launch_underfilled_to_retry(uint32_t *flags, int begin, int n, const float *thr_safe, float *thr, hipStream_t s);
int launch_scatter_thresholds(const uint32_t *list, int n, const float *thr2, float *thr, hipStream_t s);
int launch_gather_queries(const uint16_t *Q, int dim, const uint32_t *list, int n, const float *thr, const float *cq, uint16_t *Q2,
                          float *thr2, float *cq2, hipStream_t s);
int launch_dense_scores(const uint16_t *D, int dt, int64_t n_rows, int dim, const uint16_t *Q, const uint32_t *qlist,
                        int q_begin, int nq_chunk, const uint32_t *count_dev, float *out, hipStream_t s);
int launch_dense_select(const float *scores, int64_t n_rows, int k, const uint32_t *out_rows, int q_begin, int nq_chunk,
                        const uint32_t *count_dev, int64_t id_offset, float *out_scores, int64_t *out_ids, hipStream_t s,
                        bool aggregate = true, const uint32_t *in_rows = nullptr, bool in_rows_compact = false);

int launch_margin_select(const float *scores, int64_t pitch, int64_t n_rows, int k, int dim, const uint16_t *Q, const uint16_t *D, int dt,
                         const float *tile_norm, const float *row_norm, const uint32_t *dmax_bits, const float *hint, const uint32_t *out_rows,
                         int q_begin, int nq_chunk, int64_t id_offset, float *out_scores, int64_t *out_ids, uint32_t *flag_count, uint32_t *flag_list,
                         hipStream_t s);

enum SearchEvent { EV_BEGIN, EV_SAMPLE_BEGIN, EV_SAMPLE_END, EV_MAIN_BEGIN, EV_MAIN_END, EV_SELECT_END, EV_DONE, EV_ASYNC_END, EV_COUNT };

}

struct ccr_index {
    const uint16_t *D;
    int dtype;
    int64_t n_rows;
    int dim;
    int64_t offset;
    int64_t id_out;
    uint32_t *dmax_bits;
    float *tile_norm;
    size_t tile_bytes;
    const float *row_norm;
    float *row_norm_own;
    size_t row_bytes;
    bool have_events;
    int thr_phases_used;
    bool main_pass_recorded;
    int num_cu;
    int device;
    ccr::Knobs knobs;
    hipEvent_t ev[ccr::EV_COUNT];
    volatile uint32_t *host_flags;
    ccr::Plan plan;
    int plan_nq, plan_k, plan_flags;
    ccr_search_stats stats;
    struct {
        bool active;
        const uint16_t *Q;
        int n_q, k;
        float *out_scores;
        int64_t *out_ids;
        char *ws;
        hipStream_t stream;
    } pending;
};
```

### crowd-coachable-recommendations_amd/csrc/ccr_main_pass.hip

```cpp
#include "ccr_gemm_common.h"
#include "ccr_index.h"

namespace ccr {

__device__ __attribute__((aligned(16))) uint32_t g_zero_chunk[4];

__device__ __forceinline__ float load_uniform_f32(const float *p) {
    float v;
    asm volatile("s_load_dword %0, %1, 0x0\n\ts_waitcnt lgkmcnt(0)" : "=s"(v) : "s"(p) : "memory");
    return v;
}

template <int N>
__device__ __forceinline__ void wait_vm() {
    asm volatile("s_waitcnt vmcnt(%0)" ::"n"(N) : "memory");
}

typedef float f32x4v __attribute__((ext_vector_type(4)));

__device__ __forceinline__ float max4_asm(const f32x4v &c) {
    float m;
    asm("v_max3_f32 %0, %1, %2, %3\n\tv_max_f32 %0, %0, %4" : "=&v"(m) : "v"(c[0]), "v"(c[1]), "v"(c[2]), "v"(c[3]));
    return m;
}
__device__ __forceinline__ float max3_asm(float a, float b, float c) {
    float m;
    asm("v_max3_f32 %0, %1, %2, %3" : "=v"(m) : "v"(a), "v"(b), "v"(c));
    return m;
}

__device__ __forceinline__ int64_t real_tile(const GemmArgs &a, int64_t vt) {
    return a.skip_stride ? unsampled_tile(vt, a.skip_stride, a.skip_count) : vt * a.tile_stride;
}

struct ItemWalk {
    int jx, step, xcd, end;
    __device__ __forceinline__ explicit ItemWalk(const GemmArgs &a) {
        xcd = blockIdx.x & (NUM_XCD - 1);
        jx = blockIdx.x >> 3;
        step = gridDim.x >> 3;
        const int count_x = (a.ranges / NUM_XCD) * a.qblocks;
        end = a.item_end < count_x ? a.item_end : count_x;
    }
    __device__ __forceinline__ int first(const GemmArgs &a) const { return a.item_begin + jx; }
    __device__ __forceinline__ int64_t item(const GemmArgs &a, int i, int &r, int &qb) const {
        return main_item(i, xcd, a.qblocks, a.qgroups, a.qsplit, a.ranges, a.n_vt, r, qb);
    }
};


template <int ET>
struct Mfma32 {
    typedef f32x16 Acc;
    static constexpr int TILE = 32, REGS = 16, DT = 4, QT = 2, SUBLISTS = 4;
    struct Frags { bf16x8 a[2][4], b[2][2]; };

    static __device__ __forceinline__ int src_swizzle(int row) { return (row >> 2) & 3; }

    int a_base, b_base, cofs[2];
    __device__ __forceinline__ Mfma32(int lane, int wd, int wq) {
        const int swz = (lane >> 2) & 3;
#pragma unroll
        for (int ks = 0; ks < 2; ++ks) cofs[ks] = (((2 * ks + (lane >> 5)) ^ swz) << 4);
        a_base = (wd * 128 + (lane & 31)) * 64;
        b_base = SUB_Q_REGION + (wq * 64 + (lane & 31)) * 64;
    }
    __device__ __forceinline__ void read(const char *buf, Frags &f) const {
#pragma unroll
        for (int ks = 0; ks < 2; ++ks) {
#pragma unroll
            for (int dt = 0; dt < 4; ++dt) f.a[ks][dt] = *reinterpret_cast<const bf16x8 *>(buf + a_base + dt * 2048 + cofs[ks]);
#pragma unroll
            for (int qt = 0; qt < 2; ++qt) f.b[ks][qt] = *reinterpret_cast<const bf16x8 *>(buf + b_base + qt * 2048 + cofs[ks]);
        }
    }
    static __device__ __forceinline__ void mma(Acc (&acc)[4][2], const Frags &f, bool first) {
        if (first) {
            const f32x16 z = {0.f, 0.f, 0.f, 0.f, 0.f, 0.f, 0.f, 0.f, 0.f, 0.f, 0.f, 0.f, 0.f, 0.f, 0.f, 0.f};
#pragma unroll
            for (int dt = 0; dt < 4; ++dt)
#pragma unroll
                for (int qt = 0; qt < 2; ++qt) acc[dt][qt] = mfma_32x32x16<ET>(f.a[0][dt], f.b[0][qt], z);
        } else {
#pragma unroll
            for (int dt = 0; dt < 4; ++dt)
#pragma unroll
                for (int qt = 0; qt < 2; ++qt) acc[dt][qt] = mfma_32x32x16<ET>(f.a[0][dt], f.b[0][qt], acc[dt][qt]);
        }
#pragma unroll
        for (int dt = 0; dt < 4; ++dt)
#pragma unroll
            for (int qt = 0; qt < 2; ++qt) acc[dt][qt] = mfma_32x32x16<ET>(f.a[1][dt], f.b[1][qt], acc[dt][qt]);
    }

    static __device__ __forceinline__ void tile_max(const Acc (&acc)[4][2], int qt, float (&sub)[4][4], float (&mdt)[4]) {
#pragma unroll
        for (int dt = 0; dt < 4; ++dt) {
#pragma unroll
            for (int g = 0; g < 4; ++g)
                sub[dt][g] = fmaxf(fmaxf(acc[dt][qt][4 * g], acc[dt][qt][4 * g + 1]), fmaxf(acc[dt][qt][4 * g + 2], acc[dt][qt][4 * g + 3]));
            mdt[dt] = fmaxf(fmaxf(sub[dt][0], sub[dt][1]), fmaxf(sub[dt][2], sub[dt][3]));
        }
    }
    static __device__ __forceinline__ void gmax(const Acc (&acc)[4][2], const GemmArgs &a, int64_t vt, int q0, int wd, int wq, int lane) {
        const int h = lane >> 5;
#pragma unroll
        for (int qt = 0; qt < 2; ++qt) {
            float sub[4][4], mdt[4];
            tile_max(acc, qt, sub, mdt);
            const int ql = wq * 64 + qt * 32 + (lane & 31);
#pragma unroll
            for (int dt = 0; dt < 4; ++dt) a.gmax[(vt * GROUPS_PER_TILE + wd * 8 + dt * 2 + h) * a.nq_pad + q0 + ql] = mdt[dt];
        }
    }
    static __device__ __forceinline__ void filter(const Acc (&acc)[4][2], const float (&thr)[2], const float (&cqv)[2], float nt,
                                                  int64_t row_base, const GemmArgs &a, uint2 *const (&clist)[2], uint32_t (&ncand)[2],
                                                  int cap) {
        const uint32_t row32 = (uint32_t)row_base;
        const int64_t left = a.n_rows - row_base;
        const uint32_t rows_left = left <= 0 ? 0u : (left > 128 ? 128u : (uint32_t)left);
#pragma unroll
        for (int qt = 0; qt < 2; ++qt) {
            float sub[4][4], mdt[4];
            tile_max(acc, qt, sub, mdt);
            const float t = fmaf(-cqv[qt], nt, thr[qt]);
            const float mall = fmaxf(fmaxf(mdt[0], mdt[1]), fmaxf(mdt[2], mdt[3]));
            if (__ballot(mall >= t) == 0ull) continue;
#pragma unroll
            for (int dt = 0; dt < 4; ++dt) {
                if (__ballot(mdt[dt] >= t) == 0ull) continue;
#pragma unroll
                for (int g = 0; g < 4; ++g) {
                    if (sub[dt][g] >= t) {
#pragma unroll
                        for (int e2 = 0; e2 < 4; ++e2) {
                            const float v = acc[dt][qt][4 * g + e2];
                            const uint32_t off = (uint32_t)(dt * 32 + 8 * g + e2);
                            if (v >= t && off < rows_left) {
                                if (ncand[qt] < (uint32_t)cap) clist[qt][ncand[qt] * 4] = make_uint2(__float_as_uint(v), row32 + off);
                                ++ncand[qt];
                            }
                        }
                    }
                }
            }
        }
    }
};

template <int ET>
struct Mfma16 {
    typedef f32x4v Acc;
    static constexpr int TILE = 16, REGS = 4, DT = 8, QT = 4, SUBLISTS = 8;
    struct Frags { bf16x8 a[8], b[4]; };

    static __device__ __forceinline__ int src_swizzle(int row) { return ((row >> 2) & 1) << 1; }

    int a_base, b_base;
    __device__ __forceinline__ Mfma16(int lane, int wd, int wq) {
        const int cofs = (((lane >> 4) ^ (((lane >> 2) & 1) << 1)) << 4);
        a_base = (wd * 128 + (lane & 15)) * 64 + cofs;
        b_base = SUB_Q_REGION + (wq * 64 + (lane & 15)) * 64 + cofs;
    }
    __device__ __forceinline__ void read(const char *buf, Frags &f) const {
#pragma unroll
        for (int dt = 0; dt < 8; ++dt) f.a[dt] = *reinterpret_cast<const bf16x8 *>(buf + a_base + dt * 1024);
#pragma unroll
        for (int qt = 0; qt < 4; ++qt) f.b[qt] = *reinterpret_cast<const bf16x8 *>(buf + b_base + qt * 1024);
    }
    static __device__ __forceinline__ void mma(Acc (&acc)[8][4], const Frags &f, bool first) {
        if (first) {
            const f32x4v z = {0.f, 0.f, 0.f, 0.f};
#pragma unroll
            for (int dt = 0; dt < 8; ++dt)
#pragma unroll
                for (int qt = 0; qt < 4; ++qt) acc[dt][qt] = mfma_16x16x32<ET>(f.a[dt], f.b[qt], z);
            return;
        }
#pragma unroll
        for (int dt = 0; dt < 8; ++dt)
#pragma unroll
            for (int qt = 0; qt < 4; ++qt) acc[dt][qt] = mfma_16x16x32<ET>(f.a[dt], f.b[qt], acc[dt][qt]);
    }

    static __device__ __forceinline__ void filter(const Acc (&acc)[8][4], const float (&thr)[4], const float (&cqv)[4], float nt,
                                                  int64_t row_base, const GemmArgs &a, uint2 *const (&clist)[4], uint32_t (&ncand)[4],
                                                  int cap) {
#pragma unroll
        for (int qt = 0; qt < 4; ++qt) {
            float sub[8];
#pragma unroll
            for (int dt = 0; dt < 8; ++dt) sub[dt] = max4_asm(acc[dt][qt]);
            const float t = fmaf(-cqv[qt], nt, thr[qt]);
            float mall = max3_asm(sub[0], sub[1], sub[2]);
            mall = max3_asm(mall, sub[3], sub[4]);
            mall = max3_asm(mall, sub[5], sub[6]);
            mall = fmaxf(mall, sub[7]);
            if (__ballot(mall >= t) == 0ull) continue;
#pragma unroll
            for (int dt = 0; dt < 8; ++dt) {
                if (sub[dt] >= t) {
#pragma unroll
                    for (int e = 0; e < 4; ++e) {
                        const float v = acc[dt][qt][e];
                        const int64_t doc = row_base + dt * 16 + e;
                        if (v >= t && doc < a.n_rows) {
                            if (ncand[qt] < (uint32_t)cap) clist[qt][ncand[qt] * 8] = make_uint2(__float_as_uint(v), (uint32_t)doc);
                            ++ncand[qt];
                        }
                    }
                }
            }
        }
    }
};

template <class S, int EPI, bool TAIL>
__device__ __forceinline__ void main_pass_256(const GemmArgs &a) {
    static_assert(EPI != EPI_GMAX || S::TILE == 32, "EPI_GMAX exists on the 32x32 shape only");
    extern __shared__ __attribute__((aligned(16))) char smem[];

    const int tid = threadIdx.x & (GEMM_THREADS - 1);
    const int lane = tid & 63;
    const int wv = __builtin_amdgcn_readfirstlane(tid >> 6);
    const int wd = wv >> 2;
    const int wq = wv & 3;
    const int lc = lane & (S::TILE - 1);
    const int lh = lane / S::TILE;
    const int cell = wd * (S::SUBLISTS / 2) + lh;
    const bool g1 = (wv >= 4);
    const int KS2 = TAIL ? (a.dim + SUB_K - 1) / SUB_K : a.dim / SUB_K;

    const int srow = wv * 16 + (lane >> 2);
    const int schunk = (lane & 3) ^ S::src_swizzle(srow);
    const S mfma(lane, wd, wq);

    const ItemWalk walk(a);
    for (int item = walk.first(a); item < walk.end; item += walk.step) {
        int r, qb;
        const int64_t ntile = walk.item(a, item, r, qb);
        if (ntile <= 0) continue;
        const int q0 = qb * TILE_Q;

        float thr[S::QT] = {}, cqv[S::QT] = {};
        uint32_t ncand[S::QT] = {};
        uint2 *clist[S::QT] = {};
        int cap = 0;
        if (EPI == EPI_FILTER) {
            int seg_r0;
            long long seg_base;
            cand_segment(a.lay, r, cap, seg_r0, seg_base);
#pragma unroll
            for (int qt = 0; qt < S::QT; ++qt) {
                const int q = q0 + wq * 64 + qt * S::TILE + lc;
                thr[qt] = (q < a.n_q) ? a.thr[q] : __builtin_nanf("");
                cqv[qt] = (q < a.n_q) ? a.cq[q] : 0.f;
                clist[qt] = a.cand + seg_base + ((int64_t)(r - seg_r0) * a.nq_pad + q) * S::SUBLISTS * cap + cell;
            }
#pragma unroll
            for (int qt = 0; qt < S::QT; ++qt) asm volatile("" : "+v"(thr[qt]), "+v"(cqv[qt]));
        }
        float *dst[S::QT] = {};
        if (EPI == EPI_STORE) {
            const int64_t pitch = a.store_pitch ? a.store_pitch : a.n_rows;
#pragma unroll
            for (int qt = 0; qt < S::QT; ++qt) {
                const int q = q0 + wq * 64 + qt * S::TILE + lc;
                if (q < a.n_q) dst[qt] = a.store + (int64_t)q * pitch;
            }
        }
        const uint16_t *qsrc[2];
#pragma unroll
        for (int i = 0; i < 2; ++i) {
            int qrow = q0 + i * 128 + srow;
            if (qrow > a.n_q - 1) qrow = a.n_q - 1;
            qsrc[i] = a.Q + (int64_t)qrow * a.dim + schunk * 8;
        }

        typename S::Acc acc[S::DT][S::QT];
        const int64_t U = ntile * KS2;

        int64_t iu = 0, it = 0;
        int iks = 0;
        const uint16_t *dsrc[2];
        auto tile_ptrs = [&]() {
            const int64_t row0 = real_tile(a, r + it * a.ranges) * TILE_DOCS;
#pragma unroll
            for (int i = 0; i < 2; ++i) {
                int64_t drow = row0 + (i * 128 + srow);
                if (drow > a.n_rows - 1) drow = a.n_rows - 1;
                dsrc[i] = a.D + drow * a.dim + schunk * 8;
            }
        };
        tile_ptrs();
        auto issue = [&]() {
            char *buf = smem + (int)(iu & (RING - 1)) * SUB_BYTES;
            const int k0 = iks * SUB_K;
            if (TAIL && iks == KS2 - 1) {
                const bool in = k0 + schunk * 8 < a.dim;
#pragma unroll
                for (int i = 0; i < 2; ++i)
                    glds16(in ? (const void *)(dsrc[i] + k0) : (const void *)g_zero_chunk, buf + (i * 512 + wv * 64) * 16);
#pragma unroll
                for (int i = 0; i < 2; ++i)
                    glds16(in ? (const void *)(qsrc[i] + k0) : (const void *)g_zero_chunk, buf + SUB_Q_REGION + (i * 512 + wv * 64) * 16);
            } else {
#pragma unroll
                for (int i = 0; i < 2; ++i) glds16(dsrc[i] + k0, buf + (i * 512 + wv * 64) * 16);
#pragma unroll
                for (int i = 0; i < 2; ++i) glds16(qsrc[i] + k0, buf + SUB_Q_REGION + (i * 512 + wv * 64) * 16);
            }
            ++iu;
            if (++iks == KS2) {
                iks = 0;
                ++it;
                tile_ptrs();
            }
        };

        auto epilogue = [&](int64_t vt, int64_t rt, float nt) {
            const int64_t row_base = rt * TILE_DOCS + wd * 128 + 4 * lh;
            if constexpr (EPI == EPI_GMAX) {
                S::gmax(acc, a, vt, q0, wd, wq, lane);
            } else if constexpr (EPI == EPI_FILTER) {
                S::filter(acc, thr, cqv, nt, row_base, a, clist, ncand, cap);
            } else {
                const int64_t pitch = a.store_pitch ? a.store_pitch : a.n_rows;
#pragma unroll
                for (int qt = 0; qt < S::QT; ++qt) {
                    if (!dst[qt]) continue;
#pragma unroll
                    for (int dt = 0; dt < S::DT; ++dt)
#pragma unroll
                        for (int g = 0; g < S::REGS / 4; ++g) {
                            const int64_t doc = row_base + dt * S::TILE + 8 * g;
                            if ((pitch & 3) == 0 && doc + 3 < a.n_rows) {
                                *reinterpret_cast<float4 *>(dst[qt] + doc) = make_float4(acc[dt][qt][4 * g], acc[dt][qt][4 * g + 1],
                                                                                             acc[dt][qt][4 * g + 2], acc[dt][qt][4 * g + 3]);
                            } else {
#pragma unroll
                                for (int e2 = 0; e2 < 4; ++e2)
                                    if (doc + e2 < a.n_rows) dst[qt][doc + e2] = acc[dt][qt][4 * g + e2];
                            }
                        }
                }
            }
        };

        const int npro = U < 3 ? (int)U : 3;
        for (int i = 0; i < npro; ++i) issue();
        if (npro == 3)
            CCR_WAIT_VM(8);
        else if (npro == 2)
            CCR_WAIT_VM(4);
        else
            CCR_WAIT_VM(0);
        CCR_BARRIER();
        if (g1) CCR_BARRIER();

        int cks = 0;
        int64_t ct = 0;
        bool pending = false;
        int64_t pending_vt = 0, pending_rt = 0;
        float pending_nt = 0.f;
        for (int64_t u = 0; u < U; ++u) {
            if (pending) {
                epilogue(pending_vt, pending_rt, pending_nt);
                pending = false;
            }
            if (u + 1 < U) {
                if (u + 2 < U)
                    CCR_WAIT_VM(4);
                else
                    CCR_WAIT_VM(0);
            }
            typename S::Frags f;
            mfma.read(smem + (int)(u & (RING - 1)) * SUB_BYTES, f);
            if (u + 3 < U) issue();
            CCR_WAIT_LGKM0();
            CCR_BARRIER();
            S::mma(acc, f, cks == 0);
            if (++cks == KS2) {
                cks = 0;
                const int64_t vt_done = r + ct * a.ranges;
                const int64_t rt_done = real_tile(a, vt_done);
                const float nt_done = EPI == EPI_FILTER ? load_uniform_f32(a.tile_norm + rt_done) : 0.f;
                if (g1) {
                    epilogue(vt_done, rt_done, nt_done);
                } else {
                    pending = true;
                    pending_vt = vt_done;
                    pending_rt = rt_done;
                    pending_nt = nt_done;
                }
                ++ct;
            }
            CCR_BARRIER();
        }
        if (pending) epilogue(pending_vt, pending_rt, pending_nt);
        if (!g1) CCR_BARRIER();

        if (EPI == EPI_FILTER) {
#pragma unroll
            for (int qt = 0; qt < S::QT; ++qt)
                a.cnt[((int64_t)r * a.nq_pad + q0 + wq * 64 + qt * S::TILE + lc) * S::SUBLISTS + cell] = ncand[qt];
        }
        __syncthreads();
    }
}

template <int ET, int EPI, bool TAIL = false>
__global__ __launch_bounds__(GEMM_THREADS, 2) void gemm_topk_kernel(const GemmArgs a) { main_pass_256<Mfma32<ET>, EPI, TAIL>(a); }
template <int ET, int EPI, bool TAIL = false>
__global__ __launch_bounds__(GEMM_THREADS, 2) void gemm_topk16_kernel(const GemmArgs a) { main_pass_256<Mfma16<ET>, EPI, TAIL>(a); }


__device__ __forceinline__ int fresh_lane() {
    int l;
    asm volatile("v_mbcnt_lo_u32_b32 %0, -1, 0\n\tv_mbcnt_hi_u32_b32 %0, -1, %0" : "=v"(l));
    return l;
}
__device__ __forceinline__ uint32_t lds_offset(const void *p) {
    return (uint32_t)(uintptr_t)(const __attribute__((address_space(3))) void *)p;
}
template <int OFF>
__device__ __forceinline__ uint64_t lds_issue_read_b64(uint32_t addr) {
    uint64_t v;
    asm volatile("ds_read_b64 %0, %1 offset:%2" : "=v"(v) : "v"(addr), "n"(OFF) : "memory");
    return v;
}
template <int OFF>
__device__ __forceinline__ uint32_t lds_issue_read_b32(uint32_t addr) {
    uint32_t v;
    asm volatile("ds_read_b32 %0, %1 offset:%2" : "=v"(v) : "v"(addr), "n"(OFF) : "memory");
    return v;
}
template <int OFF>
__device__ __forceinline__ void lds_issue_write_b32(uint32_t addr, uint32_t v) {
    asm volatile("ds_write_b32 %0, %1 offset:%2" ::"v"(addr), "v"(v), "n"(OFF) : "memory");
}
__device__ __forceinline__ void lds_wait_cells(uint64_t (&tc)[6], uint32_t (&cn)[6]) {
    asm volatile("s_waitcnt lgkmcnt(0)"
                 : "+v"(tc[0]), "+v"(tc[1]), "+v"(tc[2]), "+v"(tc[3]), "+v"(tc[4]), "+v"(tc[5]), "+v"(cn[0]), "+v"(cn[1]), "+v"(cn[2]), "+v"(cn[3]),
                   "+v"(cn[4]), "+v"(cn[5])
                 :
                 : "memory");
}
constexpr int WIDE_SUB_BYTES = (TILE_DOCS + WIDE_Q) * SUB_K * 2;
constexpr int WIDE_Q_REGION = TILE_DOCS * SUB_K * 2;
constexpr int WIDE_RING = 3;
constexpr int WIDE_PIECES = 5;
constexpr int WIDE_QT = 6;
constexpr int WIDE_RING_BYTES = WIDE_RING * WIDE_SUB_BYTES;
constexpr size_t WIDE_LDS = (size_t)WIDE_RING_BYTES + WIDE_Q * 8 + (size_t)(GEMM_THREADS / 64) * WIDE_QT * 64 * 4;

template <int ET>
__global__ __launch_bounds__(GEMM_THREADS, 2) void gemm_topk16w_kernel(const GemmArgs a) {
    extern __shared__ __attribute__((aligned(16))) char smem[];
    float2 *s_tc = reinterpret_cast<float2 *>(smem + WIDE_RING_BYTES);
    uint32_t *s_cnt = reinterpret_cast<uint32_t *>(smem + WIDE_RING_BYTES + WIDE_Q * 8);
    const int wv = __builtin_amdgcn_readfirstlane((int)threadIdx.x >> 6);
    const int wd = wv >> 2;
    const int wq = wv & 3;
    const bool g1 = (wv >= 4);
    const int KS2 = a.dim / SUB_K;
    const uint32_t pitch = (uint32_t)a.dim * 2u;
    uint32_t lane_src, lane_lds;
    {
        const int ln = fresh_lane();
        const int pr = ln >> 2;
        lane_src = (uint32_t)pr * pitch + (uint32_t)(((ln & 3) ^ (((pr >> 2) & 1) << 1)) << 4);
        lane_lds = (uint32_t)((ln & 15) * 64 + (((ln >> 4) ^ (((ln >> 2) & 1) << 1)) << 4));
    }

    const ItemWalk walk(a);
    for (int item = walk.first(a); item < walk.end; item += walk.step) {
        int r, qb;
        const int64_t ntile = walk.item(a, item, r, qb);
        if (ntile <= 0) continue;
        const int q0 = qb * WIDE_Q;

        int cap, seg_r0;
        long long seg_base;
        cand_segment(a.lay, r, cap, seg_r0, seg_base);
        {
            const int ln = fresh_lane();
            const int tid = wv * 64 + ln;
            if (tid < WIDE_Q) {
                const int q = q0 + tid;
                s_tc[tid] = make_float2((q < a.n_q) ? a.thr[q] : __builtin_nanf(""), (q < a.n_q) ? a.cq[q] : 0.f);
            }
#pragma unroll
            for (int qt = 0; qt < WIDE_QT; ++qt) s_cnt[(wv * WIDE_QT + qt) * 64 + ln] = 0u;
        }
        CCR_WAIT_VM(0);

        const int qlimit = (a.n_q - 1 - q0 < WIDE_Q - 1) ? a.n_q - 1 - q0 : WIDE_Q - 1;
        const char *qblk = reinterpret_cast<const char *>(a.Q) + (int64_t)q0 * pitch;

        f32x4v acc[8][WIDE_QT];
        const int U = (int)(ntile * KS2);
        int islot = 0, iks = 0;
        int64_t it = 0;
        const char *dtile = nullptr;
        int dlimit = 0;
        auto tile_base = [&]() __attribute__((always_inline)) {
            const int64_t row0 = real_tile(a, r + it * a.ranges) * TILE_DOCS;
            dlimit = (a.n_rows - 1 - row0 < TILE_DOCS - 1) ? (int)(a.n_rows - 1 - row0) : TILE_DOCS - 1;
            dtile = reinterpret_cast<const char *>(a.D) + row0 * pitch;
        };
        tile_base();
        const bool q_whole = g1 ? ((wv - 4) * 96 + 95 <= qlimit) : (wv * 96 + 15 <= qlimit);
        auto issue = [&]() __attribute__((always_inline)) {
            char *buf = smem + islot * WIDE_SUB_BYTES;
            const uint32_t kb = (uint32_t)iks * (SUB_K * 2);
            if (q_whole && (g1 || dlimit == TILE_DOCS - 1)) {
                const uint32_t voff = lane_src + kb;
                if (!g1) {
                    const char *rows = dtile + (size_t)(wv * 64) * pitch;
#pragma unroll
                    for (int i = 0; i < 4; ++i) glds16(rows + (size_t)(i * 16) * pitch + voff, buf + (wv * 4 + i) * 1024);
                    glds16(qblk + (size_t)(wv * 96) * pitch + voff, buf + WIDE_Q_REGION + wv * 96 * 64);
                } else {
                    const char *rows = qblk + (size_t)((wv - 4) * 96 + 16) * pitch;
                    char *dst = buf + WIDE_Q_REGION + ((wv - 4) * 96 + 16) * 64;
#pragma unroll
                    for (int i = 0; i < WIDE_PIECES; ++i) glds16(rows + (size_t)(i * 16) * pitch + voff, dst + i * 1024);
                }
            } else {
                const int iln = fresh_lane();
                const int pr = iln >> 2;
                const uint32_t co = (uint32_t)(((iln & 3) ^ (((pr >> 2) & 1) << 1)) << 4) + kb;
                auto piece = [&](const char *rows, int row0, int limit, char *dst) __attribute__((always_inline)) {
                    int row = row0 + pr;
                    row = row < limit ? row : limit;
                    glds16(rows + ((uint32_t)row * pitch + co), dst);
                };
                if (!g1) {
#pragma unroll
                    for (int i = 0; i < 4; ++i) piece(dtile, (wv * 4 + i) * 16, dlimit, buf + (wv * 4 + i) * 1024);
                    piece(qblk, wv * 96, qlimit, buf + WIDE_Q_REGION + wv * 96 * 64);
                } else {
#pragma unroll
                    for (int i = 0; i < WIDE_PIECES; ++i)
                        piece(qblk, (wv - 4) * 96 + 16 * (1 + i), qlimit, buf + WIDE_Q_REGION + ((wv - 4) * 96 + 16 * (1 + i)) * 64);
                }
            }
            islot = islot == WIDE_RING - 1 ? 0 : islot + 1;
            if (++iks == KS2) {
                iks = 0;
                ++it;
                if (!g1) tile_base();
            }
        };

        auto epilogue = [&](int64_t rt, float nt) __attribute__((always_inline)) {
            const int eln = fresh_lane();
            const int l15o = eln & 15, lqo = eln >> 4;
            char *const cbase = reinterpret_cast<char *>(a.cand + seg_base + ((int64_t)(r - seg_r0) * a.nq_pad + q0) * 8 * cap + wd * 4);
            const uint32_t row_lo = (uint32_t)(wd * 128 + 4 * lqo);
            const uint32_t tc_addr = lds_offset(s_tc) + (uint32_t)(wq * 96 + l15o) * 8u;
            const uint32_t cnt_addr = lds_offset(s_cnt) + (uint32_t)(wv * WIDE_QT * 64 + lqo * 16 + l15o) * 4u;
            const int64_t tile_row0 = rt * TILE_DOCS;
            const uint32_t rows_left = a.n_rows - tile_row0 < TILE_DOCS ? (uint32_t)(a.n_rows - tile_row0) : (uint32_t)TILE_DOCS;
            uint64_t tcr[WIDE_QT];
            uint32_t cnr[WIDE_QT];
            tcr[0] = lds_issue_read_b64<0 * 128>(tc_addr);
            tcr[1] = lds_issue_read_b64<1 * 128>(tc_addr);
            tcr[2] = lds_issue_read_b64<2 * 128>(tc_addr);
            tcr[3] = lds_issue_read_b64<3 * 128>(tc_addr);
            tcr[4] = lds_issue_read_b64<4 * 128>(tc_addr);
            tcr[5] = lds_issue_read_b64<5 * 128>(tc_addr);
            cnr[0] = lds_issue_read_b32<0 * 256>(cnt_addr);
            cnr[1] = lds_issue_read_b32<1 * 256>(cnt_addr);
            cnr[2] = lds_issue_read_b32<2 * 256>(cnt_addr);
            cnr[3] = lds_issue_read_b32<3 * 256>(cnt_addr);
            cnr[4] = lds_issue_read_b32<4 * 256>(cnt_addr);
            cnr[5] = lds_issue_read_b32<5 * 256>(cnt_addr);
            float sub0[8];
#pragma unroll
            for (int dt = 0; dt < 8; ++dt) sub0[dt] = max4_asm(acc[dt][0]);
            __builtin_amdgcn_sched_barrier(0);
            lds_wait_cells(tcr, cnr);
#pragma unroll
            for (int qt = 0; qt < WIDE_QT; ++qt) {
                float sub[8];
#pragma unroll
                for (int dt = 0; dt < 8; ++dt) sub[dt] = qt == 0 ? sub0[dt] : max4_asm(acc[dt][qt]);
                const float t = fmaf(-__uint_as_float((uint32_t)(tcr[qt] >> 32)), nt, __uint_as_float((uint32_t)tcr[qt]));
                float mall = max3_asm(sub[0], sub[1], sub[2]);
                mall = max3_asm(mall, sub[3], sub[4]);
                mall = max3_asm(mall, sub[5], sub[6]);
                mall = fmaxf(mall, sub[7]);
                if (__ballot(mall >= t) != 0ull) {
                    const uint32_t ql = (uint32_t)(wq * 96 + qt * 16 + l15o);
                    const uint32_t cell = (ql * 8u * (uint32_t)cap + (uint32_t)lqo) * 8u;
#pragma unroll
                    for (int dt = 0; dt < 8; ++dt) {
                        if (sub[dt] >= t) {
#pragma unroll
                            for (int e = 0; e < 4; ++e) {
                                const float v = acc[dt][qt][e];
                                const uint32_t row = row_lo + dt * 16 + e;
                                if (v >= t && row < rows_left) {
                                    const uint32_t n = cnr[qt]++;
                                    if (n < (uint32_t)cap)
                                        *reinterpret_cast<uint2 *>(cbase + (cell + n * 64u)) = make_uint2(__float_as_uint(v), (uint32_t)tile_row0 + row);
                                }
                            }
                        }
                    }
                }
            }
            lds_issue_write_b32<0 * 256>(cnt_addr, cnr[0]);
            lds_issue_write_b32<1 * 256>(cnt_addr, cnr[1]);
            lds_issue_write_b32<2 * 256>(cnt_addr, cnr[2]);
            lds_issue_write_b32<3 * 256>(cnt_addr, cnr[3]);
            lds_issue_write_b32<4 * 256>(cnt_addr, cnr[4]);
            lds_issue_write_b32<5 * 256>(cnt_addr, cnr[5]);
        };

        const int npro = U < 2 ? U : 2;
        for (int i = 0; i < npro; ++i) issue();
        if (npro == 2)
            wait_vm<WIDE_PIECES>();
        else
            CCR_WAIT_VM(0);
        CCR_BARRIER();
        if (g1) CCR_BARRIER();

        int cks = 0;
        int64_t ct = 0;
        bool pending = false;
        int64_t pending_rt = 0;
        float pending_nt = 0.f;
        int uslot = 0;
        for (int u = 0; u < U; ++u) {
            if (u + 2 < U) issue();
            __builtin_amdgcn_sched_barrier(0);
            if (pending) {
                epilogue(pending_rt, pending_nt);
                pending = false;
            }
            const char *abuf = smem + uslot * WIDE_SUB_BYTES;
            const char *bbuf = abuf + WIDE_Q_REGION;
            uslot = uslot == WIDE_RING - 1 ? 0 : uslot + 1;
            const int a_base = wd * 128 * 64 + (int)lane_lds;
            const int b_base = wq * 96 * 64 + (int)lane_lds;
            bf16x8 af[8], bfr[WIDE_QT];
#pragma unroll
            for (int dt = 0; dt < 8; ++dt) af[dt] = *reinterpret_cast<const bf16x8 *>(abuf + a_base + dt * 1024);
#pragma unroll
            for (int qt = 0; qt < WIDE_QT; ++qt) bfr[qt] = *reinterpret_cast<const bf16x8 *>(bbuf + b_base + qt * 1024);
            if (u + 2 < U)
                wait_vm<WIDE_PIECES>();
            else
                CCR_WAIT_VM(0);
            CCR_WAIT_LGKM0();
            CCR_BARRIER();
            if (cks == 0) {
                const f32x4v z = {0.f, 0.f, 0.f, 0.f};
#pragma unroll
                for (int qt = 0; qt < WIDE_QT; ++qt)
#pragma unroll
                    for (int dt = 0; dt < 8; ++dt) acc[dt][qt] = mfma_16x16x32<ET>(af[dt], bfr[qt], z);
            } else {
#pragma unroll
                for (int qt = 0; qt < WIDE_QT; ++qt)
#pragma unroll
                    for (int dt = 0; dt < 8; ++dt) acc[dt][qt] = mfma_16x16x32<ET>(af[dt], bfr[qt], acc[dt][qt]);
            }
            if (++cks == KS2) {
                cks = 0;
                const int64_t rt_done = real_tile(a, r + ct * a.ranges);
                const float nt_done = load_uniform_f32(a.tile_norm + rt_done);
                if (g1) {
                    epilogue(rt_done, nt_done);
                } else {
                    pending = true;
                    pending_rt = rt_done;
                    pending_nt = nt_done;
                }
                ++ct;
            }
            CCR_WAIT_LGKM0();
            CCR_BARRIER();
        }
        if (pending) epilogue(pending_rt, pending_nt);
        CCR_WAIT_LGKM0();
        if (!g1) CCR_BARRIER();

        {
            const int ln = fresh_lane();
#pragma unroll
            for (int qt = 0; qt < WIDE_QT; ++qt)
                a.cnt[((int64_t)r * a.nq_pad + q0 + wq * 96 + qt * 16 + (ln & 15)) * 8 + wd * 4 + (ln >> 4)] = s_cnt[(wv * WIDE_QT + qt) * 64 + ln];
        }
        __syncthreads();
    }
}

template <class K>
static int launch_kernel(K kernel, size_t lds, const GemmArgs &a, int grid, hipStream_t s) {
    const int rc = ensure_dynamic_lds(reinterpret_cast<const void *>(kernel), lds);
    if (rc != CCR_OK) return rc;
    hipLaunchKernelGGL(kernel, dim3(grid), dim3(GEMM_THREADS), lds, s, a);
    CCR_LAUNCH_CHECK();
    return CCR_OK;
}

template <int ET>
static int launch_gemm_of(const GemmArgs &a, MainKernel kind, int epi, int grid, hipStream_t s) {
    if (epi != EPI_FILTER && epi != EPI_GMAX && epi != EPI_STORE) {
        set_error("launch_gemm: unknown epilogue %d", epi);
        return CCR_ERR_INVALID;
    }
    if (kind == MAIN_WIDE) {
        if (epi != EPI_FILTER || a.dim % SUB_K != 0 || a.dim < SUB_K) {
            set_error("launch_gemm: the 256 x 384 kernel takes EPI_FILTER and dim %% %d == 0 only (epi %d, dim %d)", SUB_K, epi, a.dim);
            return CCR_ERR_INVALID;
        }
        return launch_kernel(&gemm_topk16w_kernel<ET>, WIDE_LDS, a, grid, s);
    }
    typedef void (*Kernel)(const GemmArgs);
    static const Kernel k256[2][3][2] = {
        {{gemm_topk_kernel<ET, EPI_FILTER>, gemm_topk_kernel<ET, EPI_FILTER, true>},
         {gemm_topk_kernel<ET, EPI_GMAX>, gemm_topk_kernel<ET, EPI_GMAX, true>},
         {gemm_topk_kernel<ET, EPI_STORE>, gemm_topk_kernel<ET, EPI_STORE, true>}},
        {{gemm_topk16_kernel<ET, EPI_FILTER>, gemm_topk16_kernel<ET, EPI_FILTER, true>},
         {nullptr, nullptr},
         {gemm_topk16_kernel<ET, EPI_STORE>, gemm_topk16_kernel<ET, EPI_STORE, true>}},
    };
    const Kernel k = k256[kind == MAIN_16X16][epi][a.dim % SUB_K != 0];
    if (!k) {
        set_error("launch_gemm: the 16x16x32 kernel has no EPI_GMAX");
        return CCR_ERR_INVALID;
    }
    return launch_kernel(k, RING * (size_t)SUB_BYTES, a, grid, s);
}

int launch_gemm(const GemmArgs &a, int dt, MainKernel kind, int epi, int grid, hipStream_t s) {
    return dispatch_half(dt, [&](auto et) { return launch_gemm_of<decltype(et)::value>(a, kind, epi, grid, s); });
}

}
```

### crowd-coachable-recommendations_amd/csrc/ccr_plan.h

```cpp
#pragma once
#include "ccr_common.h"
#include "ccr_narrow.h"

namespace ccr {

struct Knobs {
    int qgroups;
    int progressive;
    int max_phases;
    int mfma16;
    int sample_div;
    int ranges;
    int optimistic;
    int opt_rank;
    int max_lists;
    int narrow;
    int narrow_grid;
    int skip_sampled;
    int skip_list;
    int qsplit;
    int wide;
    int thr_phases;
    int narrow_groups;
    int tile_cap;
};
struct KnobDef {
    const char *env;
    int Knobs::*field;
    int dflt;
};
inline constexpr KnobDef KNOB_DEFS[] = {
    {"CCR_QGROUPS", &Knobs::qgroups, 0},           {"CCR_PROGRESSIVE", &Knobs::progressive, 1},   {"CCR_PHASES", &Knobs::max_phases, 3},
    {"CCR_MFMA16", &Knobs::mfma16, -1},            {"CCR_SAMPLE_DIV", &Knobs::sample_div, 0},     {"CCR_RANGES", &Knobs::ranges, 0},
    {"CCR_OPTIMISTIC", &Knobs::optimistic, -1},    {"CCR_OPT_RANK", &Knobs::opt_rank, 0},         {"CCR_MAX_LISTS", &Knobs::max_lists, 0},
    {"CCR_NARROW", &Knobs::narrow, -1},            {"CCR_NARROW_GRID", &Knobs::narrow_grid, 0},   {"CCR_SKIP_SAMPLED", &Knobs::skip_sampled, -1},
    {"CCR_SKIP_LIST", &Knobs::skip_list, 1},       {"CCR_QSPLIT", &Knobs::qsplit, -1},            {"CCR_WIDE", &Knobs::wide, -1},
    {"CCR_THR_PHASES", &Knobs::thr_phases, 0},     {"CCR_NARROW_GROUPS", &Knobs::narrow_groups, NARROW_MAX_GROUPS},
    {"CCR_TILE_CAP", &Knobs::tile_cap, 0},
};
static_assert(sizeof(KNOB_DEFS) / sizeof(KNOB_DEFS[0]) * sizeof(int) == sizeof(Knobs), "a row for every knob");
inline Knobs default_knobs() {
    Knobs kn;
    for (const KnobDef &d : KNOB_DEFS) kn.*d.field = d.dflt;
    return kn;
}
Knobs read_knobs();

struct Plan {
    int fused;
    int nq_pad;
    int qblocks;
    int tile_q;
    int main_qblocks;
    int main_qgroups;
    int main_qsplit;
    int64_t tiles;
    int64_t full_tiles;
    int sample_tiles;
    int64_t sample_stride;
    int sample_ranges;
    int ranges;
    int item_a;
    int item_b;
    int opt_rank;
    int tile_cap;
    int cap_rank;
    int skip_sampled;
    int qgroups;
    int cap;
    CandLayout cand;
    int grid;
    int rescore_cap;
    int rescore_regular;
    int select_compact;
    int mfma16;
    int sublists;
    int narrow;
    int narrow_groups;
    int first_nsub;
    int first_sp;
    CandLayout first_lay;
    int64_t cand_recs;
    size_t total;
    int64_t dense_rows_per_chunk;
};

constexpr int TILE_CAP_MIN = 4, TILE_CAP_TILES = 5;
constexpr int OPT_RANK_MIN = TILE_CAP_MIN * (TILE_CAP_TILES - 1) + 1;
constexpr int OPT_RANK_FLOOR = 40, REDUCED_RANK_MIN_TILES = 40;

constexpr int FALLBACK_ROWS = 16;

Plan make_plan(int64_t n_rows, int dim, int n_q, int k, int flags, int num_cu, const Knobs &kn);

inline int64_t round_up(int64_t v, int64_t m) { return (v + m - 1) / m * m; }
int pick_qgroups(int qblocks, int dim, const Knobs &kn, int tile_q = TILE_Q);
CandLayout one_segment(int cap);

struct Bump {
    size_t off;
    size_t take(size_t bytes) { const size_t o = off; off = (off + bytes + 255) / 256 * 256; return o; }
};

struct SearchWs {
    float *qnorm, *thr, *cq, *gmax;
    uint32_t *cnt;
    uint2 *cand;
    uint32_t *flag_count, *flag_list;
    unsigned long long *stat_cand;
    uint32_t *top;
    float *thr_safe, *cq_safe, *dense;
    uint32_t *glist;
    uint16_t *Q2;
    float *thr2, *cq2;
    uint32_t *retry_list, *dense_list, *counts, *flag2, *list_b, *list_c;
    size_t cand_bytes, dense_bytes, retry_bytes, total;
};
SearchWs search_ws(const Plan &p, int64_t n_rows, int dim, int n_q, int k, char *base);
inline int skip_list_cap(int opt_rank) { return 2 * opt_rank + 30; }

}
```

### crowd-coachable-recommendations_amd/csrc/ccr_plan.hip

```cpp
#include <stdlib.h>
#include <string.h>

#include <math.h>

#include <algorithm>
#include <vector>

#include "ccr_index.h"
#include "ccr_topk_device.h"

namespace ccr {

Knobs read_knobs() {
    Knobs kn = default_knobs();
    for (const KnobDef &d : KNOB_DEFS)
        if (const char *e = getenv(d.env)) kn.*d.field = atoi(e);
    return kn;
}

constexpr double L2_RESIDENT_BYTES = 3.2 * 1048576.0, L2_MOSTLY_BYTES = 5.5 * 1048576.0;
constexpr double WIDE_TILE_COST = 1.37;
constexpr double MODEL_QUERIES = 3584.0;

static double tile_cost(const Plan &p) { return p.tile_q == WIDE_Q ? WIDE_TILE_COST : 1.0; }
static double query_scale(const Plan &p) { return (double)p.nq_pad / MODEL_QUERIES; }

static double gamma_upper(double r) { return 1.25 * (r + 4.75 * sqrt(r) + 8.0) / r; }

static double estimated_pass(int rank, double fs, int k) { return std::max((double)rank / fs, (double)k); }
static double sample_fraction(const Plan &p) { return 1.0 / ((double)p.tiles / (double)p.sample_tiles); }
static double estimated_pass_upper(const Plan &p, int k) {
    return gamma_upper((double)p.cap_rank) * estimated_pass(p.cap_rank, sample_fraction(p), k);
}
static double conservative_pass(const Plan &p, int k) { return (double)k * ((double)p.tiles / (double)p.sample_tiles) * 1.3 + 64.0; }

int pick_qgroups(int qblocks, int dim, const Knobs &kn, int tile_q) {
    {
        const int v = kn.qgroups;
        if ((v == 1 || v == 2 || v == 4 || v == 8) && qblocks % v == 0) return v;
    }
    const size_t block_bytes = (size_t)tile_q * dim * 2;
    int best = 1;
    for (int gq = 1; gq <= NUM_XCD; gq *= 2) {
        if (qblocks % gq) continue;
        best = gq;
        if ((size_t)(qblocks / gq) * block_bytes <= (size_t)3 << 20) break;
    }
    return best;
}

static int footprint_class(double bytes) { return bytes <= L2_RESIDENT_BYTES ? 0 : (bytes <= L2_MOSTLY_BYTES ? 1 : 2); }

static int pick_qsplit(int qblocks, int equal_groups, int dim, int tile_q, const Knobs &kn) {
    if (kn.qsplit == 0) return 0;
    const int v = kn.qgroups;
    if (v == 2 || v == 4 || v == 8) return qblocks % v ? v : 0;
    const double block_bytes = (double)tile_q * dim * 2.0;
    const int equal_class = footprint_class((double)(qblocks / equal_groups) * block_bytes);
    for (int G = 2; G <= NUM_XCD; G *= 2)
        if (qblocks % G && footprint_class((double)(qblocks / G + qblocks % G) * block_bytes) < equal_class) return G;
    if (kn.qsplit == 1)
        for (int G = 2; G <= NUM_XCD; G *= 2)
            if (qblocks % G) return G;
    return 0;
}

static int best_sample_ranges(int64_t n_vt, int qblocks, int qgroups, int grid) {
    const int nrc = NUM_XCD / qgroups, qb_per = qblocks / qgroups, per_x = std::max(1, grid / NUM_XCD);
    int best_r = NUM_XCD;
    double best = 1e300;
    const int64_t r_max = round_up(std::min<int64_t>(n_vt, 1024), NUM_XCD);
    std::vector<double> load((size_t)per_x);
    for (int64_t R = NUM_XCD; R <= r_max; R += NUM_XCD) {
        double worst = 0.0;
        for (int rc = 0; rc < nrc; ++rc) {
            std::fill(load.begin(), load.end(), 0.0);
            const int64_t items = R / nrc * qb_per;
            for (int64_t item = 0; item < items; ++item) {
                const int64_t r = rc + nrc * (item / qb_per);
                const int64_t ntile = (n_vt - r + R - 1) / R;
                if (ntile > 0) load[(size_t)(item % per_x)] += (double)ntile + 0.15;
            }
            worst = std::max(worst, *std::max_element(load.begin(), load.end()));
        }
        if (worst < best - 1e-9) {
            best = worst;
            best_r = (int)R;
        }
    }
    return best_r;
}

constexpr size_t DENSE_SCRATCH_TARGET = (size_t)1 << 30;

struct MainPassChoice {
    int64_t sample, ranges;
    int item_a, item_b;
    int opt_rank;
    int skip;
};

static bool may_skip_sampled(const Plan &p, int64_t sample, const Knobs &kn) {
    if (kn.skip_sampled == 0 || p.narrow || sample < 1) return false;
    const int64_t stride = std::max<int64_t>(1, p.full_tiles / sample);
    return stride >= 2 && (sample - 1) * stride < p.full_tiles && sample < p.tiles;
}

static int optimistic_rank(int k, int64_t sample, int64_t tiles, const Knobs &kn, bool skip = false) {
    if (kn.opt_rank > 0) return kn.opt_rank;
    const double need = (double)k * (double)sample / (double)(skip ? tiles - sample : tiles);
    int r = (skip && sample >= REDUCED_RANK_MIN_TILES) ? OPT_RANK_MIN : OPT_RANK_FLOOR;
    for (; r < 1 << 20; ++r) {
        const double a = 1.0 / (9.0 * r), t = 1.0 - a - 5.2 * sqrt(a);
        if (t > 0.0 && (double)r * t * t * t >= need) break;
    }
    return r;
}

static int tile_cap_for(int rank, int64_t sample, const Knobs &kn) {
    int cap = (rank + TILE_CAP_TILES - 1) / TILE_CAP_TILES;
    cap = std::min(GROUPS_PER_TILE, std::max(TILE_CAP_MIN, cap));
    if (kn.tile_cap >= 1 && kn.tile_cap <= GROUPS_PER_TILE) cap = kn.tile_cap;
    const int64_t fill = ((int64_t)rank + sample - 1) / std::max<int64_t>(1, sample);
    return (int)std::min<int64_t>(GROUPS_PER_TILE, std::max<int64_t>(cap, fill));
}

static void range_window(const Plan &p, const Knobs &kn, int64_t &r_hi, int64_t &target) {
    int64_t max_lists = p.rescore_cap > 512 ? 2048 : 1024;
    if ((max_lists / p.sublists) * p.main_qblocks < p.grid) max_lists = 2048;
    if (kn.max_lists >= 64 && kn.max_lists < max_lists) max_lists = kn.max_lists;
    r_hi = std::min<int64_t>(max_lists / p.sublists, round_up(std::max<int64_t>(1, p.tiles / 8), NUM_XCD));
    target = std::min<int64_t>(r_hi, round_up(std::max<int64_t>(NUM_XCD, (int64_t)p.grid * 6 / p.main_qblocks), NUM_XCD));
}

static double sample_cost(const Plan &p, int64_t smp) {
    return (double)((smp * p.qblocks + p.grid - 1) / p.grid) + 0.015 * (double)smp * std::max(1.0, query_scale(p));
}

struct Best {
    double cost;
    MainPassChoice choice;
    void offer(double c, const MainPassChoice &ch) {
        if (c < cost) cost = c, choice = ch;
    }
};

static void price_range_count(const Plan &p, int k, const Knobs &kn, int64_t smp, int64_t R, int64_t target, bool reprice_skipped, Best &best) {
    const int nrc = NUM_XCD / p.main_qgroups, qb_per = p.main_qblocks / p.main_qgroups, per_x = p.grid / NUM_XCD;
    const double qscale = query_scale(p);
    const double select_per_range = 0.1 * qscale, hit_w = 0.014 * qscale, phase_w = 3.0;
    const double fs = (double)smp / (double)p.tiles;
    auto survivors = [&](double fa, double fb) -> double {
        if (fa <= 0.0) return (double)k / fs;
        if (fb <= 0.0) return (double)k * (fa / fs + (1.0 - fa) / fa);
        return (double)k * (fa / fs + fb / fa + (1.0 - fa - fb) / (fa + fb));
    };
    const int64_t items = R / nrc * qb_per;
    const double item_cost = ((double)((p.tiles + R - 1) / R) + 0.15) * tile_cost(p);
    auto rounds = [&](int64_t n) { return (double)((n + per_x - 1) / per_x); };
    const double common = sample_cost(p, smp) + select_per_range * (double)R + 1e-3 * std::abs((double)(R - target));
    const double single = rounds(items) * item_cost + hit_w * survivors(0.0, 0.0) + common;
    if (kn.optimistic != 1 && !reprice_skipped) best.offer(single, {smp, R, 0, 0, 0, 0});
    if (kn.optimistic != 0 && smp * GROUPS_PER_TILE >= 160) {
        const bool skip = reprice_skipped && may_skip_sampled(p, smp, kn);
        const int rank = optimistic_rank(k, smp, p.tiles, kn, skip);
        if ((int64_t)rank * 4 <= smp * GROUPS_PER_TILE) {
            const double opt_item = skip ? ((double)((p.tiles - smp + R - 1) / R) + 0.15) * tile_cost(p) : item_cost;
            const double opt = rounds(items) * opt_item + hit_w * estimated_pass(rank, fs, k) + common - (kn.optimistic == 1 ? 1e9 : 0.0);
            best.offer(opt, {smp, R, 0, 0, rank, skip ? 1 : 0});
        }
    }
    if (reprice_skipped || kn.progressive == 0 || p.narrow || !(items > per_x && (double)p.tiles / (double)R >= 8.0)) return;
    const double fa = (double)per_x / (double)items;
    best.offer((1.0 + rounds(items - per_x)) * item_cost + phase_w + hit_w * survivors(fa, 0.0) + common, {smp, R, per_x, 0, 0, 0});
    if (kn.max_phases < 3) return;
    for (int ph = 1; ph <= 3; ++ph) {
        const int64_t ib = (int64_t)per_x * (1 + ph);
        if (ib >= items) break;
        const double fb = (double)ph * per_x / (double)items;
        best.offer((1.0 + ph + rounds(items - ib)) * item_cost + 2.0 * phase_w + hit_w * survivors(fa, fb) + common, {smp, R, per_x, (int)ib, 0, 0});
    }
}

static MainPassChoice choose_main_pass(const Plan &p, int k, const std::vector<int64_t> &samples, const Knobs &kn, bool reprice_skipped = false) {
    int64_t r_hi, target;
    range_window(p, kn, r_hi, target);
    Best best = {1e300, {samples[0], target, 0, 0, 0, 0}};
    const int64_t r_lo = std::max<int64_t>(NUM_XCD, target / 2 / NUM_XCD * NUM_XCD);
    for (int64_t smp : samples)
        for (int64_t R = r_lo; R <= std::min(r_hi, target * 2); R += NUM_XCD) {
            if (kn.ranges > 0 && R != std::min<int64_t>(r_hi, std::max<int64_t>(r_lo, round_up(kn.ranges, NUM_XCD)))) continue;
            price_range_count(p, k, kn, smp, R, target, reprice_skipped, best);
        }
    return best.choice;
}

struct Search {
    int64_t n_rows;
    int dim, n_q, k, flags, num_cu;
    const Knobs &kn;
};

static int64_t sample_for(const Plan &p, int k, int64_t div) {
    const int64_t min_sample = (2 * (int64_t)k + GROUPS_PER_TILE - 1) / GROUPS_PER_TILE;
    return std::max<int64_t>({(p.tiles + div - 1) / div, min_sample, 4});
}
static bool sample_div_forced(const Knobs &kn) { return kn.sample_div >= 4 && kn.sample_div <= 256; }
static int64_t sample_div(const Knobs &kn) { return sample_div_forced(kn) ? kn.sample_div : 32; }

static Plan plan_geometry(const Search &s, int mfma16) {
    Plan p;
    memset(&p, 0, sizeof(p));
    p.nq_pad = (int)round_up(s.n_q, TILE_Q);
    p.qblocks = p.nq_pad / TILE_Q;
    p.tile_q = TILE_Q;
    p.main_qblocks = p.qblocks;
    p.main_qgroups = 1;
    p.tiles = (s.n_rows + TILE_DOCS - 1) / TILE_DOCS;
    p.full_tiles = s.n_rows / TILE_DOCS;
    p.grid = std::max(NUM_XCD, s.num_cu / NUM_XCD * NUM_XCD);
    p.mfma16 = mfma16;
    p.sublists = p.mfma16 ? 8 : 4;
    p.rescore_cap = p.rescore_regular = std::min(8192, std::max(256, 2 * pow2_ceil(s.k)));
    return p;
}

static int64_t decide_fused(const Search &s, Plan &p) {
    int64_t sample = sample_for(p, s.k, sample_div(s.kn));
    bool fused = (s.dim % 8 == 0) && s.dim >= 8 && (sample * 4 <= p.full_tiles) && s.k <= MAX_K;
    if ((s.flags & CCR_SEARCH_FORCE_FUSED) && (s.dim % 8 == 0) && p.full_tiles >= 1) {
        if (!fused) sample = std::min<int64_t>(std::max<int64_t>(sample, 1), p.full_tiles);
        fused = sample * GROUPS_PER_TILE >= s.k;
    }
    if (s.flags & CCR_SEARCH_FORCE_DENSE) fused = false;
    p.fused = fused ? 1 : 0;
    return sample;
}

static std::vector<int64_t> sample_sizes(const Search &s, const Plan &p, int64_t sample) {
    const bool pinned = sample_div_forced(s.kn) || (s.flags & CCR_SEARCH_FORCE_FUSED);
    const int64_t sample_alt = pinned ? sample : sample_for(p, s.k, 2 * sample_div(s.kn));
    int64_t sample_big = pinned ? sample : sample_for(p, s.k, sample_div(s.kn) / 2);
    if (sample_big * 4 > p.full_tiles) sample_big = sample;
    std::vector<int64_t> sizes = {sample};
    for (int64_t v : {sample_alt, sample_big})
        if (std::find(sizes.begin(), sizes.end(), v) == sizes.end()) sizes.push_back(v);
    return sizes;
}

static void choose_streaming(const Search &s, Plan &p) {
    const Knobs &kn = s.kn;
    const int n_q = s.n_q, dim = s.dim;
    int nqt = n_q <= 16 ? 1 : (n_q <= 32 ? 2 : 4);
    int ngroups = n_q <= NARROW_MAX_Q ? 1 : 2;
    if (n_q > NARROW_MAX_Q && n_q <= 96 && kn.narrow_groups >= 2 && dim % TILE_K == 0 && narrow_lds_bytes(6, dim) <= (size_t)160 * 1024)
        nqt = 6, ngroups = 1;
    const bool narrow = kn.narrow != 0 && n_q <= NARROW_MAX_Q * std::min(std::max(kn.narrow_groups, 1), NARROW_MAX_GROUPS) && dim % TILE_K == 0 &&
                        narrow_lds_bytes(nqt, dim) <= (size_t)160 * 1024 && (ngroups == 1 || s.num_cu >= 16);
    p.narrow = narrow ? nqt : 0;
    p.narrow_groups = narrow ? ngroups : 1;
}

static void choose_tile(const Search &s, Plan &p) {
    const Knobs &kn = s.kn;
    const int n_q = s.n_q, dim = s.dim;
    if (!p.narrow && p.mfma16 && dim % 32 == 0 && kn.wide != 0) {
        static const double per_flop_of_class[3] = {0.95, 0.97, 1.04};
        const int wb = (n_q + WIDE_Q - 1) / WIDE_Q;
        const double per_xcd = (double)(wb / pick_qgroups(wb, dim, kn, WIDE_Q)) * WIDE_Q * dim * 2.0;
        const double per_flop = per_flop_of_class[footprint_class(per_xcd)];
        if (kn.wide == 1 || (double)wb * WIDE_Q * per_flop < (double)p.qblocks * TILE_Q) {
            p.tile_q = WIDE_Q;
            p.main_qblocks = wb;
            p.nq_pad = (int)round_up(std::max<int64_t>(n_q, (int64_t)wb * WIDE_Q), TILE_Q);
            p.qblocks = p.nq_pad / TILE_Q;
            p.qgroups = pick_qgroups(p.qblocks, dim, kn);
        }
    }
    p.main_qgroups = pick_qgroups(p.main_qblocks, dim, kn, p.tile_q);
}

static void set_rank_dependents(Plan &p, const Knobs &kn) {
    p.tile_cap = p.opt_rank > 0 ? tile_cap_for(p.opt_rank, p.sample_tiles, kn) : GROUPS_PER_TILE;
    p.cap_rank = (kn.opt_rank > 0 || p.opt_rank == 0) ? p.opt_rank : std::max(p.opt_rank, OPT_RANK_FLOOR);
}

static void choose_launches(const Search &s, Plan &p, const std::vector<int64_t> &samples) {
    const Knobs &kn = s.kn;
    MainPassChoice choice = choose_main_pass(p, s.k, samples, kn);
    if (choice.opt_rank > 0 && may_skip_sampled(p, choice.sample, kn)) {
        const MainPassChoice skipped = choose_main_pass(p, s.k, {choice.sample}, kn, true);
        if (skipped.skip) choice = skipped;
    }
    p.sample_tiles = (int)choice.sample;
    p.sample_stride = std::max<int64_t>(1, p.full_tiles / choice.sample);
    p.sample_ranges = best_sample_ranges(choice.sample, p.qblocks, p.qgroups, p.grid);
    p.ranges = (int)choice.ranges;
    p.item_a = choice.item_a;
    p.item_b = choice.item_b;
    p.opt_rank = choice.opt_rank;
    set_rank_dependents(p, kn);
    p.skip_sampled = (p.opt_rank > 0 && !p.narrow) ? choice.skip : 0;
    p.main_qsplit = (!p.narrow && p.item_a == 0 && p.item_b == 0) ? pick_qsplit(p.main_qblocks, p.main_qgroups, s.dim, p.tile_q, kn) : 0;
}

static void price_skip_sampled(const Search &s, Plan &p) {
    if (!p.skip_sampled) return;
    const int k = s.k;
    const double join_rows = 256.0 * (double)p.sample_tiles * (1.0 - pow(1.0 - std::min(1.0, (double)k / (double)s.n_rows), 16.0));
    const double need = (double)k + (double)(k / 4) + 1.5 * join_rows + TILE_DOCS + 16;
    const double saved = 0.5 * (double)p.sample_tiles * p.main_qblocks * tile_cost(p) / (double)p.grid;
    const bool pays = 0.065 * join_rows * query_scale(p) < saved;
    if (need > 8192.0 || (s.kn.skip_sampled < 0 && !pays)) {
        p.skip_sampled = 0;
        p.opt_rank = std::max(p.opt_rank, optimistic_rank(k, p.sample_tiles, p.tiles, s.kn, false));
        set_rank_dependents(p, s.kn);
    } else
        p.rescore_cap = std::min(8192, std::max(p.rescore_cap, pow2_ceil((int)need)));
}

CandLayout one_segment(int cap) {
    CandLayout L;
    memset(&L, 0, sizeof(L));
    L.nseg = 1;
    L.seg_end[0] = L.seg_end[1] = L.seg_end[2] = INT32_MAX;
    L.cap[0] = L.cap[1] = L.cap[2] = cap;
    return L;
}

static void plan_candidates(const Search &s, Plan &p) {
    const int k = s.k;
    const int64_t R = p.ranges;
    const int nrc_p = NUM_XCD / p.main_qgroups, qb_per_p = p.main_qblocks / p.main_qgroups;
    auto ranges_to = [&](int item) { return item ? std::min<int64_t>(R, (int64_t)nrc_p * ((item + qb_per_p - 1) / qb_per_p)) : 0; };
    const int64_t RA = ranges_to(p.item_a), RB = ranges_to(p.item_b);
    const double fs = sample_fraction(p), nlists = (double)R * p.sublists;
    const double xk = gamma_upper((double)k);
    const int64_t tile_rows = TILE_DOCS / p.sublists;
    auto cap_for = [&](double g) -> int {
        const double mean = p.opt_rank ? estimated_pass_upper(p, k) / nlists : xk * (double)k / (g * nlists);
        const int64_t c = (int64_t)(mean + 6.0 * sqrt(mean)) + 16 + tile_rows;
        return (int)round_up(std::min<int64_t>(std::max<int64_t>(c, 16), 8192), 4);
    };
    const double fa = p.item_a ? (double)(p.item_a / qb_per_p) * nrc_p / (double)R : 0.0;
    const double fb = p.item_b ? std::max(0.0, (double)(p.item_b / qb_per_p) * nrc_p / (double)R - fa) : 0.0;
    const double upd_compact = std::min(32768.0, std::max(4096.0, 8.0 * pow2_ceil(k)));
    auto seen = [&](double g, double found) { return found > upd_compact ? g * upd_compact / found : g; };
    const double found_a = (double)k * fa / fs;
    CandLayout &L = p.cand;
    memset(&L, 0, sizeof(L));
    const int seg_end_v[3] = {RA ? (int)RA : (int)R, RB > RA ? (int)RB : (int)R, (int)R};
    int64_t recs = 0;
    int prev_end = 0;
    for (int g = 0; g < 3; ++g) L.seg_end[g] = INT32_MAX, L.cap[g] = 16;
    for (int g = 0; g < 3; ++g) {
        if (seg_end_v[g] <= prev_end) continue;
        const int sg = L.nseg++;
        double frac_seen = fs;
        if (sg == 1) frac_seen = fa >= 2.0 * fs ? seen(fa, found_a) : fs;
        if (sg == 2) frac_seen = fa >= 2.0 * fs ? seen(fa + fb, found_a + (double)k * fb / fa) : fs;
        L.seg_end[sg] = seg_end_v[g];
        L.cap[sg] = cap_for(std::min(1.0, std::max(frac_seen, fs)));
        L.base[sg] = recs;
        recs += (int64_t)(seg_end_v[g] - prev_end) * p.nq_pad * p.sublists * L.cap[sg];
        recs = round_up(recs, 32);
        prev_end = seg_end_v[g];
    }
    L.seg_end[L.nseg - 1] = INT32_MAX;
    p.cap = L.cap[0];
    p.cand_recs = recs;
}

static void plan_select_and_first_pass(const Search &s, Plan &p) {
    const int k = s.k, n_q = s.n_q;
    const double expect = conservative_pass(p, k);
    double want = expect;
    if (p.opt_rank)
        want = std::max(estimated_pass_upper(p, k) + 512.0, k > 256 ? 18.0 * k : 0.0);
    else if (p.item_a)
        want = 16.0 * k + 512.0;
    p.select_compact = select_compact_entries(s.dim, p.ranges * p.sublists, p.rescore_cap, (int64_t)(want * 1.25));
    p.first_nsub = p.ranges * p.sublists;
    p.first_sp = p.sublists;
    p.first_lay = p.cand;
    if (p.narrow) {
        const double pass = p.opt_rank ? estimated_pass_upper(p, k) : expect;
        int64_t capn = std::max<int64_t>(p.cand_recs / ((int64_t)NARROW_SUBLISTS * std::max(1, n_q)), (int64_t)(8.0 * pass) + 4096);
        capn = std::min<int64_t>(capn, (int64_t)1 << 22) / 4 * 4;
        p.cand_recs = std::max<int64_t>(p.cand_recs, capn * NARROW_SUBLISTS * n_q);
        p.first_lay = one_segment((int)capn);
        p.first_nsub = NARROW_SUBLISTS;
        p.first_sp = NARROW_SUBLISTS;
    }
}

static int64_t dense_chunk_rows(const Search &s) {
    int64_t rows = (int64_t)(DENSE_SCRATCH_TARGET / ((size_t)s.n_rows * 4));
    rows = std::min<int64_t>(std::max<int64_t>(rows, 1), s.n_q);
    if (rows >= 64) rows = rows / 64 * 64;
    return rows;
}

static Plan make_plan_for(const Search &s, int mfma16) {
    Plan p = plan_geometry(s, mfma16);
    const int64_t sample = decide_fused(s, p);
    if (p.fused) {
        p.qgroups = pick_qgroups(p.qblocks, s.dim, s.kn);
        const std::vector<int64_t> samples = sample_sizes(s, p, sample);
        choose_streaming(s, p);
        choose_tile(s, p);
        choose_launches(s, p, samples);
        price_skip_sampled(s, p);
        plan_candidates(s, p);
        plan_select_and_first_pass(s, p);
        p.dense_rows_per_chunk = FALLBACK_ROWS;
    } else {
        p.dense_rows_per_chunk = dense_chunk_rows(s);
    }
    p.total = search_ws(p, s.n_rows, s.dim, s.n_q, s.k, nullptr).total;
    return p;
}

SearchWs search_ws(const Plan &p, int64_t n_rows, int dim, int n_q, int k, char *base) {
    SearchWs w;
    memset(&w, 0, sizeof(w));
    Bump b = {0};
    auto at = [&](size_t off) { return (char *)((uintptr_t)base + off); };
    auto take = [&](size_t bytes) { return at(b.take(bytes)); };
    if (!p.fused) {
        w.flag_count = (uint32_t *)take(64 + (size_t)n_q * 4);
        w.flag_list = w.flag_count + 16;
        w.dense_bytes = (size_t)p.dense_rows_per_chunk * (n_rows + 3) * 4;
        w.dense = (float *)take(w.dense_bytes);
        w.total = b.off;
        return w;
    }
    const size_t nq_pad = p.nq_pad;
    w.qnorm = (float *)take(nq_pad * 4);
    w.thr = (float *)take(nq_pad * 8);
    w.cq = w.thr + nq_pad;
    w.gmax = (float *)take((size_t)p.sample_tiles * GROUPS_PER_TILE * nq_pad * 4);
    w.cnt = (uint32_t *)take((size_t)p.ranges * nq_pad * p.sublists * 4);
    w.cand = (uint2 *)take((size_t)p.cand_recs * 8);
    w.flag_count = (uint32_t *)take(64 + (size_t)n_q * 4);
    w.stat_cand = (unsigned long long *)(w.flag_count + 2);
    w.flag_list = w.flag_count + 16;
    w.cand_bytes = (char *)w.flag_count - (char *)w.cand;
    w.top = (uint32_t *)take(p.item_b ? (nq_pad + (size_t)n_q * k) * 4 : 0);
    w.thr_safe = (float *)take(p.opt_rank ? nq_pad * 8 : 0);
    w.cq_safe = w.thr_safe + nq_pad;
    w.glist = (uint32_t *)take(p.skip_sampled ? nq_pad * (size_t)(skip_list_cap(p.opt_rank) + 1) * 4 : 0);
    w.dense_bytes = (size_t)p.dense_rows_per_chunk * n_rows * 4;
    w.dense = (float *)take(w.dense_bytes);
    w.retry_bytes = nq_pad * dim * 2 + nq_pad * 8 + (size_t)n_q * 16 + 64 + 64 + (size_t)n_q * 4 + 256 * 10;
    Bump r = {b.take(w.retry_bytes)};
    w.Q2 = (uint16_t *)at(r.take(nq_pad * dim * 2));
    w.thr2 = (float *)at(r.take(nq_pad * 4));
    w.cq2 = (float *)at(r.take(nq_pad * 4));
    w.retry_list = (uint32_t *)at(r.take((size_t)n_q * 4));
    w.dense_list = (uint32_t *)at(r.take((size_t)n_q * 4));
    w.counts = (uint32_t *)at(r.take(64));
    w.flag2 = (uint32_t *)at(r.take(64 + (size_t)n_q * 4));
    w.list_b = (uint32_t *)at(r.take((size_t)n_q * 4));
    w.list_c = (uint32_t *)at(r.take((size_t)n_q * 4));
    w.total = b.off;
    return w;
}

Plan make_plan(int64_t n_rows, int dim, int n_q, int k, int flags, int num_cu, const Knobs &kn) {
    const Search s = {n_rows, dim, n_q, k, flags, num_cu, kn};
    if (kn.mfma16 >= 0) return make_plan_for(s, kn.mfma16 ? 1 : 0);
    if (k <= 512) return make_plan_for(s, 1);
    const Plan p32 = make_plan_for(s, 0);
    if (p32.fused && p32.ranges * 8 <= 2048) return make_plan_for(s, 1);
    return p32;
}

}
```

### include/ccr_retrieval.h

```cpp
#ifndef CCR_RETRIEVAL_H
#define CCR_RETRIEVAL_H

#include <stddef.h>
#include <stdint.h>

#ifdef __cplusplus
extern "C" {
#endif

#define CCR_OK 0
#define CCR_ERR_INVALID (-1)
#define CCR_ERR_HIP (-2)
#define CCR_ERR_WORKSPACE (-3)
#define CCR_ERR_BLOCK_ID (-4)

#define CCR_DTYPE_F32 0
#define CCR_DTYPE_F16 1
#define CCR_DTYPE_BF16 2

#define CCR_SEARCH_DEFAULT 0
#define CCR_SEARCH_FORCE_DENSE 1
#define CCR_SEARCH_FORCE_FUSED 2
#define CCR_SEARCH_ASYNC 4

#define CCR_SCORES_CANONICAL 0
#define CCR_SCORES_MFMA 1

typedef struct ccr_index ccr_index;

typedef struct ccr_search_stats {
    int32_t path;
    int32_t n_fallback;
    int32_t sample_tiles;
    int32_t ranges;
    int32_t cap;
    int32_t sublists;
    int64_t n_candidates;
    float ms_sample;
    float ms_threshold;
    float ms_main;
    float ms_select;
    float ms_fallback;
    float ms_total;
    int32_t n_retried;
    int32_t n_dense;
    int32_t main_launches;
    int32_t opt_rank;
    int32_t main_tile_queries;
    int32_t skipped_tiles;
    int32_t tile_cap;
} ccr_search_stats;

const char *ccr_last_error(void);
int ccr_version(void);

int ccr_pack_bf16(const float *src, uint16_t *dst, float *norms, int64_t rows, int dim, int normalize, void *stream);
int ccr_pack_bf16_ex(const float *src, uint16_t *dst, float *norms, float *row_norm_bounds, int64_t rows, int dim, int normalize,
                     void *stream);

int ccr_pack_bf16_padded(const float *src, int64_t rows, int src_dim, uint16_t *dst, int dst_dim, float *norms,
                         float *row_norm_bounds, int normalize, void *stream);

int ccr_meanpool_pack_bf16(const void *hidden, int hidden_dtype, const int64_t *mask, uint16_t *dst_bf16,
                           float *dst_f32, int B, int L, int dim, int normalize, void *stream);
int ccr_meanpool_pack_bf16_ex(const void *hidden, int hidden_dtype, const int64_t *mask, uint16_t *dst_bf16,
                              float *dst_f32, const int64_t *dst_rows, float *row_norm_bounds, int B, int L, int dim,
                              int normalize, void *stream);

int ccr_meanpool_pack_bf16_packed(const void *hidden, int hidden_dtype, const int32_t *seq_start, const int32_t *seq_len,
                                  uint16_t *dst_bf16, float *dst_f32, const int64_t *dst_rows, float *row_norm_bounds, int n_seq,
                                  int dim, int normalize, void *stream);

int ccr_pack_half_ex(const float *src, uint16_t *dst, float *norms, float *row_norm_bounds, int64_t rows, int dim, int normalize,
                     int half_dtype, int32_t *overflow, void *stream);
int ccr_pack_half_padded(const float *src, int64_t rows, int src_dim, uint16_t *dst, int dst_dim, float *norms, float *row_norm_bounds,
                         int normalize, int half_dtype, int32_t *overflow, void *stream);
int ccr_meanpool_pack_half_ex(const void *hidden, int hidden_dtype, const int64_t *mask, uint16_t *dst_half, float *dst_f32,
                              const int64_t *dst_rows, float *row_norm_bounds, int B, int L, int dim, int normalize, int half_dtype,
                              int32_t *overflow, void *stream);
int ccr_meanpool_pack_half_packed(const void *hidden, int hidden_dtype, const int32_t *seq_start, const int32_t *seq_len,
                                  uint16_t *dst_half, float *dst_f32, const int64_t *dst_rows, float *row_norm_bounds, int n_seq, int dim,
                                  int normalize, int half_dtype, int32_t *overflow, void *stream);

int ccr_meanpool_bwd(const float *grad, const int64_t *mask, void *dhidden, int hidden_dtype, int B, int L, int dim,
                     void *stream);

int ccr_embed_layernorm(const float *word_table, int64_t vocab, const float *position_table, int64_t n_positions,
                        const float *type_table, int64_t n_types, const int64_t *token_ids, const int64_t *positions,
                        const int64_t *token_types, const float *gamma, const float *beta, float eps, float *out_f32,
                        uint16_t *out_bf16, int64_t rows, int dim, void *stream);
int ccr_gelu_bf16(const uint16_t *x, uint16_t *y, int64_t n, void *stream);
int ccr_attention_bf16(const uint16_t *qkv, const int32_t *seq_start, const int32_t *seq_len, uint16_t *out, int n_seq,
                       int n_heads, int max_len, int pad_len, float scale, void *stream);
int ccr_add_layernorm(const uint16_t *x_bf16, const float *residual, const float *gamma, const float *beta, float eps,
                      float *out_f32, uint16_t *out_bf16, int64_t rows, int dim, void *stream);
int ccr_attention_half(const uint16_t *qkv, const int32_t *seq_start, const int32_t *seq_len, uint16_t *out, int n_seq, int n_heads,
                       int max_len, int pad_len, float scale, int half_dtype, void *stream);
int ccr_add_layernorm_half(const uint16_t *x_half, const float *residual, const float *gamma, const float *beta, float eps,
                           float *out_f32, uint16_t *out_half, int64_t rows, int dim, int half_dtype, void *stream);
int ccr_embed_layernorm_half(const float *word_table, int64_t vocab, const float *position_table, int64_t n_positions,
                             const float *type_table, int64_t n_types, const int64_t *token_ids, const int64_t *positions,
                             const int64_t *token_types, const float *gamma, const float *beta, float eps, float *out_f32,
                             uint16_t *out_half, int64_t rows, int dim, int half_dtype, void *stream);
int ccr_gelu_half(const uint16_t *x, uint16_t *y, int64_t n, int half_dtype, void *stream);
int ccr_attention_bias_half(const uint16_t *qkv, const int32_t *seq_start, const int32_t *seq_len, uint16_t *out, const float *rel_bias,
                            int R, int n_seq, int n_heads, int max_len, int pad_len, float scale, int half_dtype, void *stream);

int ccr_attention_fwd_train_half(const uint16_t *qkv, const int32_t *seq_start, const int32_t *seq_len, uint16_t *out, float *lse,
                                 int n_seq, int n_heads, int max_len, int pad_len, float scale, int half_dtype, void *stream);
size_t ccr_attention_bwd_workspace_bytes(int n_seq, int n_heads, int max_len);
int ccr_attention_bwd_half(const uint16_t *qkv, const uint16_t *out, const float *lse, const uint16_t *d_out, const int32_t *seq_start,
                           const int32_t *seq_len, uint16_t *d_qkv, int n_seq, int n_heads, int max_len, int pad_len, float scale,
                           int half_dtype, void *workspace, size_t workspace_bytes, void *stream);
int ccr_add_layernorm_bwd_half(const uint16_t *x_half, const float *residual, const float *gamma, float eps, const float *d_y,
                               float *d_res, uint16_t *d_x, float *d_gamma, float *d_beta, int64_t rows, int dim, int half_dtype,
                               void *workspace, size_t workspace_bytes, void *stream);
int ccr_gelu_bwd_half(const uint16_t *x, const uint16_t *d_y, uint16_t *d_x, int64_t n, int half_dtype, void *stream);

int ccr_dropout_bits_rows(uint32_t *bits, int64_t rows, int dim, uint64_t seed, uint32_t stream_id, double p, void *stream);
int ccr_dropout_bits_attention(uint32_t *keep_q, uint32_t *keep_k, const int32_t *seq_start, const int32_t *seq_len, int64_t n_tokens,
                               int n_seq, int n_heads, int max_len, uint64_t seed, uint32_t stream_id, double p, void *stream);
int ccr_dropout_apply(const float *x, const uint32_t *bits, float inv_keep, float *out_f32, uint16_t *out_half, int64_t rows, int dim,
                      int half_dtype, void *stream);
int ccr_attention_fwd_train_drop_half(const uint16_t *qkv, const int32_t *seq_start, const int32_t *seq_len, uint16_t *out, float *lse,
                                      const uint32_t *keep_q, float inv_keep, int n_seq, int n_heads, int max_len, int pad_len,
                                      float scale, int half_dtype, void *stream);
int ccr_attention_bwd_drop_half(const uint16_t *qkv, const uint16_t *out, const float *lse, const uint16_t *d_out,
                                const int32_t *seq_start, const int32_t *seq_len, const uint32_t *keep_q, const uint32_t *keep_k,
                                float inv_keep, uint16_t *d_qkv, int n_seq, int n_heads, int max_len, int pad_len, float scale,
                                int half_dtype, void *workspace, size_t workspace_bytes, void *stream);
int ccr_add_layernorm_drop_half(const uint16_t *x_half, const uint32_t *bits, float inv_keep, const float *residual, const float *gamma,
                                const float *beta, float eps, float *out_f32, uint16_t *out_half, int64_t rows, int dim, int half_dtype,
                                void *stream);
int ccr_add_layernorm_bwd_drop_half(const uint16_t *x_half, const uint32_t *bits, float inv_keep, const float *residual,
                                    const float *gamma, float eps, const float *d_y, float *d_res, uint16_t *d_x, float *d_gamma,
                                    float *d_beta, int64_t rows, int dim, int half_dtype, void *workspace, size_t workspace_bytes,
                                    void *stream);

int ccr_index_create(const uint16_t *D_bf16, int64_t n_rows, int dim, int64_t global_row_offset, void *stream,
                     ccr_index **out);
int ccr_index_create_with_norms(const uint16_t *D_bf16, int64_t n_rows, int dim, int64_t global_row_offset,
                                const float *row_norm_bounds, void *stream, ccr_index **out);
int ccr_index_create_half(const uint16_t *D, int64_t n_rows, int dim, int half_dtype, int64_t global_row_offset, void *stream,
                          ccr_index **out);
int ccr_index_create_with_norms_half(const uint16_t *D, int64_t n_rows, int dim, int half_dtype, int64_t global_row_offset,
                                     const float *row_norm_bounds, void *stream, ccr_index **out);
int ccr_index_destroy(ccr_index *index);
int64_t ccr_index_rows(const ccr_index *index);
int ccr_index_dim(const ccr_index *index);
int ccr_index_dtype(const ccr_index *index);

size_t ccr_search_workspace_bytes(const ccr_index *index, int n_q, int k);
int ccr_search(ccr_index *index, const uint16_t *Q_bf16, int n_q, int k, float *out_scores, int64_t *out_ids,
               void *workspace, size_t ws_bytes, int flags, void *stream);
int ccr_search_finish(ccr_index *index);
int ccr_search_last_stats(const ccr_index *index, ccr_search_stats *stats );
int ccr_search_stream_wait_main_pass(const ccr_index *index, void *stream);
int ccr_search_last_main_split(const ccr_index *index);
int ccr_search_last_threshold_phases(const ccr_index *index);

int ccr_scores(const ccr_index *index, const uint16_t *Q_bf16, int n_q, int mode, float *out, void *stream);

size_t ccr_search_blocked_workspace_bytes(const ccr_index *index, int n_q, int k, const int64_t *block_ptr_host);
int ccr_search_blocked(ccr_index *index, const uint16_t *Q_bf16, int n_q, int k, const int64_t *block_ptr_host,
                       const int64_t *block_idx, float *out_scores, int64_t *out_ids, void *workspace, size_t ws_bytes,
                       int flags, void *stream);

size_t ccr_search_sparse_prior_workspace_bytes(const ccr_index *index, int n_q, int k, const int64_t *prior_ptr_host);
int ccr_search_sparse_prior(ccr_index *index, const uint16_t *Q_bf16, int n_q, int k, const int64_t *prior_ptr_host,
                            const int64_t *prior_idx, const double *prior_val, double *out_scores, int64_t *out_ids,
                            void *workspace, size_t ws_bytes, int flags, void *stream);

int ccr_colsum_bf16(const uint16_t *X, int64_t rows, int dim, double *out , void *stream);
int ccr_colsum_half(const uint16_t *X, int64_t rows, int dim, int half_dtype, double *out , void *stream);

int ccr_merge_topk(const float *scores, const int64_t *ids, int R, int n_q, int k, float *out_scores,
                   int64_t *out_ids, void *stream);
int ccr_merge_topk_strided(const float *scores, const int64_t *ids, int64_t score_rank_stride, int64_t id_rank_stride,
                           int R, int n_q, int k, float *out_scores, int64_t *out_ids, void *stream);

#define CCR_SHARD_MAGIC 0x4d524343u
typedef struct ccr_shard_header {
    uint32_t magic;
    uint32_t n_flagged;
    uint32_t k_valid;
    uint32_t n_covered;
    int64_t row_offset;
    int64_t n_rows;
} ccr_shard_header;
size_t ccr_shard_message_bytes(int n_q, int k);
int ccr_search_shard(ccr_index *index, const uint16_t *Q_bf16, int n_q, int k, void *message, void *workspace, size_t ws_bytes,
                     int flags, void *stream);
int ccr_shard_message_fill(void *message, int n_q, int k, int k_valid, const float *scores, const int64_t *ids, int64_t row_offset,
                           int64_t n_rows, void *stream);
int ccr_merge_shard_messages(const void *messages, int64_t message_stride_bytes, int R, int n_q, int k, float *out_scores,
                             int64_t *out_ids, void *stream);
int ccr_merge_short_lists(const void *messages, int64_t message_stride_bytes, int R, int n_q, int k_list, int k_out, float *out_scores,
                          int64_t *out_ids, uint32_t *flags, uint32_t *n_flagged, void *stream);

int ccr_apply_block(const float *in_scores, const int64_t *in_ids, int n_q, int k_in, const int64_t *block_ptr,
                    const int64_t *block_idx, int64_t n_rows_total, float *out_scores, int64_t *out_ids, int k_out,
                    void *stream);

size_t ccr_inbatch_ce_workspace_bytes(int B, int dim);
int ccr_inbatch_pack3_bf16(const float *q, const float *p, const float *n, int B, int dim, uint16_t *out, void *stream);
int ccr_inbatch_ce_fwd_f32(const float *q, const float *p, const float *n, int B, int dim, float inv_temperature, uint16_t *packed,
                           float *loss, float *lse, void *workspace, size_t ws_bytes, void *stream);
int ccr_inbatch_ce_fwd(const uint16_t *Qe, const uint16_t *Pe, const uint16_t *Ne, int B, int dim,
                       float inv_temperature, float *loss, float *lse, void *workspace, size_t ws_bytes, void *stream);
int ccr_inbatch_ce_bwd(const uint16_t *Qe, const uint16_t *Pe, const uint16_t *Ne, const float *lse, int B, int dim,
                       float inv_temperature, float grad_out, float *dQ, float *dP, float *dN, void *workspace,
                       size_t ws_bytes, void *stream);
int ccr_inbatch_ce_bwd_dev(const uint16_t *Qe, const uint16_t *Pe, const uint16_t *Ne, const float *lse, int B, int dim,
                           float inv_temperature, const float *grad_out_dev, float *dQ, float *dP, float *dN,
                           void *workspace, size_t ws_bytes, void *stream);

size_t ccr_pool_ce_workspace_bytes(int n_q, int n_c, int dim);
int ccr_pool_ce_fwd(const uint16_t *Q, const uint16_t *C, const int32_t *label, const float *weight, int n_q, int n_c, int dim,
                    float inv_temperature, float *out3, float *lse, void *workspace, size_t ws_bytes, void *stream);
int ccr_pool_ce_fwd_f32(const float *q, const float *c, const int32_t *label, const float *weight, int n_q, int n_c, int dim,
                        float inv_temperature, uint16_t *packed, float *out3, float *lse, void *workspace, size_t ws_bytes,
                        void *stream);
int ccr_pool_ce_bwd_dev(const uint16_t *Q, const uint16_t *C, const int32_t *label, const float *weight, const float *lse, int n_q,
                        int n_c, int dim, float inv_temperature, const float *grad_out_dev, const float *W_dev, float *dQ, float *dC,
                        void *workspace, size_t ws_bytes, void *stream);

int ccr_bpr_sample(const int64_t *users, int B, int n_neg, int64_t n_users, const int64_t *prior_ptr, const int64_t *prior_idx,
                   const float *prior_t, float t0, const float *proposal, const double *proposal_cdf, int n_items,
                   const double *uniforms, int max_row_nnz, int64_t *out_nj, void *stream);
size_t ccr_bpr_frozen_workspace_bytes(int B, int n_neg, int dim);
int ccr_bpr_frozen_fwd(const float *table, int64_t n_rows, int dim, const float *gamma, const float *beta, float eps,
                       const int64_t *ptr_i, const int64_t *ptr_j, const int64_t *ptr_nj, const float *w, int B, int n_neg,
                       float *out3, void *workspace, size_t ws_bytes, void *stream);
int ccr_bpr_frozen_bwd_dev(const float *table, int64_t n_rows, int dim, const float *gamma, const float *beta, float eps,
                           const int64_t *ptr_i, const int64_t *ptr_j, const int64_t *ptr_nj, const float *w, int B, int n_neg,
                           const float *den_dev, const float *grad_out_dev, float *dgamma, float *dbeta, void *workspace,
                           size_t ws_bytes, void *stream);

int ccr_rank_metrics(const int64_t *ids, int n_q, int k, const int64_t *qrel_ptr, const int64_t *qrel_idx,
                     const int32_t *k_values, int n_k, float *out_rr, int32_t *out_hits, void *stream);

typedef struct ccr_bm25_index ccr_bm25_index;
int ccr_bm25_index_create(const int64_t *indptr_host, const int32_t *doc_ids, const float *tf, const double *doc_k,
                          int64_t n_terms, int64_t n_docs, double k1, ccr_bm25_index **out);
int ccr_bm25_index_destroy(ccr_bm25_index *index);
int ccr_bm25_index_set_idf(ccr_bm25_index *index, const double *idf_host, double *contrib, void *stream);
size_t ccr_bm25_search_workspace_bytes(const ccr_bm25_index *index, int n_q, int max_terms_per_query);
size_t ccr_bm25_search_workspace_bytes_k(const ccr_bm25_index *index, int n_q, int max_terms_per_query, int k);
int ccr_bm25_search_last_stats(const ccr_bm25_index *index, int64_t *out4);
int ccr_bm25_search(const ccr_bm25_index *index, const int64_t *q_ptr_host, const int32_t *q_terms_host,
                    const double *q_idf_host, int n_q, int k, float *out_scores, int64_t *out_ids, void *workspace,
                    size_t ws_bytes, void *stream);

typedef struct ccr_adamw_segment {
    float *param;
    const float *grad;
    float *exp_avg;
    float *exp_avg_sq;
    void *shadow;
    int64_t n;
    float decay, step_size, bc2_sqrt;
    int32_t shadow_dtype;
} ccr_adamw_segment;
int ccr_adamw_step(const ccr_adamw_segment *segments, int n_segments, float one_minus_beta1, float beta2, float one_minus_beta2,
                   float eps, void *stream);

typedef struct ccr_adamw_control {
    float coef;
    int32_t skip;
    float norm;
    float scale;
    int32_t growth_tracker;
    int32_t skipped_total;
    uint32_t reserved[10];
} ccr_adamw_control;
int64_t ccr_grad_stats_workspace_bytes(const ccr_adamw_segment *segments, int n_segments);
int ccr_grad_stats(const ccr_adamw_segment *segments, int n_segments, float *partials, void *stream);
int ccr_adamw_control_update(ccr_adamw_control *control, const float *partials, int64_t n_partials, float max_norm, int own_scale,
                             double growth, double backoff, int growth_interval, const float *ext_grad_scale, const float *ext_found_inf,
                             void *stream);
int ccr_adamw_step_scaled(const ccr_adamw_segment *segments, int n_segments, float one_minus_beta1, float beta2, float one_minus_beta2,
                          float eps, const ccr_adamw_control *control, void *stream);

#define CCR_EMBED_GRAD_CHUNK 64
int ccr_embed_layernorm_train_half(const float *word_table, int64_t vocab, const float *position_table, int64_t n_positions,
                                   const float *type_table, int64_t n_types, const int64_t *token_ids, const int64_t *positions,
                                   const int64_t *token_types, const float *gamma, const float *beta, float eps, const uint32_t *bits,
                                   float inv_keep, float *out_f32, uint16_t *out_half, int64_t rows, int dim, int half_dtype, void *stream);
int ccr_embed_layernorm_bwd_half(const float *word_table, int64_t vocab, const float *position_table, int64_t n_positions,
                                 const float *type_table, int64_t n_types, const int64_t *token_ids, const int64_t *positions,
                                 const int64_t *token_types, const float *gamma, float eps, const uint32_t *bits, float inv_keep,
                                 const float *d_y, float *d_x, float *d_gamma, float *d_beta, int64_t rows, int dim, void *workspace,
                                 size_t workspace_bytes, void *stream);
int ccr_embedding_grad(const int64_t *idx, const int64_t *order, const float *d_x, int64_t T, int dim, float *grad, int64_t n_rows,
                       void *stream);
int ccr_meanpool_bwd_packed(const float *grad, const int32_t *seq_start, const int32_t *seq_len, void *d_hidden, int hidden_dtype, int n_seq,
                            int dim, void *stream);

int ccr_keep_f32(const float *src, const uint16_t *half_rows, int half_dtype, int normalize, float *dst_f32, float *res_bounds, int64_t rows,
                 int dim, void *stream);
size_t ccr_rescore_f32_workspace_bytes(int n_q, int n_cand, int k, int pdim);
int ccr_rescore_f32(const float *queries_f32, const float *corpus_f32, int64_t n_rows, int pdim, const int64_t *cand_ids,
                    const float *cand_s16, int n_q, int n_cand, int k, int64_t id_offset, const float *q_norm_bounds,
                    const float *q_res_bounds, const float *corpus_max, float *out_scores, int64_t *out_ids, int32_t *flags, void *workspace,
                    size_t workspace_bytes, void *stream);

#ifdef __cplusplus
}
#endif
#endif
```

Measured before the change: 268,800.

## Reserve side CUs during main pass so a waiting stream can overlap work

Adds a planner option that shrinks the main-pass grid and leaves some CUs free when another stream has asked to wait on the main pass. The main kernel counts arriving blocks in a workspace counter, and the waiting stream runs a small gate kernel that returns once all main blocks have arrived, instead of waiting for the whole main pass to end. This lets concurrent work such as corpus packing run alongside the search. The trade-off is a slower main pass whenever CUs are carved out. A cost model decides whether carving pays off, and nothing changes unless ccr_search_stream_wait_main_pass set the hint before the search.

```diff
diff --git a/crowd-coachable-recommendations_amd/ccrec_amd/_lib.py b/crowd-coachable-recommendations_amd/ccrec_amd/_lib.py
--- a/crowd-coachable-recommendations_amd/ccrec_amd/_lib.py
+++ b/crowd-coachable-recommendations_amd/ccrec_amd/_lib.py
@@ -47,6 +47,7 @@
 AMP_OPTIM_VERSION = 110
 RANK_F32_VERSION = 111
 ATTENTION_BIAS_VERSION = 112
+SIDE_CUS_VERSION = 113
 
 SHARD_HEADER_BYTES = 32
 SHARD_MAGIC = 0x4D524343
@@ -64,7 +65,7 @@
                 ("ms_main", ctypes.c_float), ("ms_select", ctypes.c_float), ("ms_fallback", ctypes.c_float),
                 ("ms_total", ctypes.c_float), ("n_retried", ctypes.c_int32), ("n_dense", ctypes.c_int32),
                 ("main_launches", ctypes.c_int32), ("opt_rank", ctypes.c_int32), ("main_tile_queries", ctypes.c_int32),
-                ("skipped_tiles", ctypes.c_int32), ("tile_cap", ctypes.c_int32)]
+                ("skipped_tiles", ctypes.c_int32), ("tile_cap", ctypes.c_int32), ("main_grid", ctypes.c_int32), ("side_cus", ctypes.c_int32)]
 
 
 class AdamwSegment(ctypes.Structure):
diff --git a/crowd-coachable-recommendations_amd/csrc/ccr_api.hip b/crowd-coachable-recommendations_amd/csrc/ccr_api.hip
--- a/crowd-coachable-recommendations_amd/csrc/ccr_api.hip
+++ b/crowd-coachable-recommendations_amd/csrc/ccr_api.hip
@@ -72,7 +72,21 @@
 }
 
 extern "C" const char *ccr_last_error(void) { return g_err; }
-extern "C" int ccr_version(void) { return 112; }
+extern "C" int ccr_version(void) { return 113; }
+
+namespace {
+bool g_side_hint[MAX_DEVICES];
+bool side_hint_take(int device) {
+    std::lock_guard<std::mutex> lock(g_slab_mutex);
+    const bool hint = g_side_hint[device];
+    g_side_hint[device] = false;
+    return hint;
+}
+void side_hint_set(int device) {
+    std::lock_guard<std::mutex> lock(g_slab_mutex);
+    g_side_hint[device] = true;
+}
+}
 
 extern "C" int ccr_index_destroy(ccr_index *ix);
 
@@ -228,17 +242,22 @@
 
 extern "C" size_t ccr_search_workspace_bytes(const ccr_index *ix, int n_q, int k) {
     if (!ix || n_q <= 0 || k <= 0) return 0;
-    Plan a = make_plan(ix->n_rows, ix->dim, n_q, k, CCR_SEARCH_DEFAULT, ix->num_cu, ix->knobs);
-    Plan b = make_plan(ix->n_rows, ix->dim, n_q, k, CCR_SEARCH_FORCE_DENSE, ix->num_cu, ix->knobs);
-    Plan c = make_plan(ix->n_rows, ix->dim, n_q, k, CCR_SEARCH_FORCE_FUSED, ix->num_cu, ix->knobs);
-    return std::max({a.total, b.total, c.total}) + 256;
+    size_t total = make_plan(ix->n_rows, ix->dim, n_q, k, CCR_SEARCH_FORCE_DENSE, ix->num_cu, ix->knobs).total;
+    for (int flags : {CCR_SEARCH_DEFAULT, CCR_SEARCH_FORCE_FUSED})
+        for (bool side_hint : {false, true}) total = std::max(total, make_plan(ix->n_rows, ix->dim, n_q, k, flags, ix->num_cu, ix->knobs, side_hint).total);
+    return total + 256;
 }
 
 extern "C" int ccr_search_stream_wait_main_pass(const ccr_index *ix, void *stream) {
     CCR_REQUIRE(ix, "ccr_search_stream_wait_main_pass: null index");
     if (!ix->main_pass_recorded) return CCR_OK;
-    CCR_HIP_CHECK(hipStreamWaitEvent((hipStream_t)stream, ix->ev[EV_MAIN_END], 0));
-    return CCR_OK;
+    side_hint_set(ix->device);
+    if (ix->plan.side_cus == 0) {
+        CCR_HIP_CHECK(hipStreamWaitEvent((hipStream_t)stream, ix->ev[EV_MAIN_END], 0));
+        return CCR_OK;
+    }
+    CCR_HIP_CHECK(hipStreamWaitEvent((hipStream_t)stream, ix->ev[EV_MAIN_BEGIN], 0));
+    return launch_main_pass_gate(ix->side_arrive, (uint32_t)ix->plan.main_grid, (hipStream_t)stream);
 }
 
 extern "C" int ccr_search_last_stats(const ccr_index *ix, ccr_search_stats *stats) {
@@ -393,7 +412,8 @@
         gm.item_begin = done;
         gm.item_end = bounds[ph];
         const MainKernel kind = p.tile_q == WIDE_Q ? MAIN_WIDE : p.mfma16 ? MAIN_16X16 : MAIN_32X32;
-        const int rc = launch_gemm(gm, ix->dtype, kind, EPI_FILTER, p.grid, s);
+        gm.arrive = p.side_cus ? w.arrive : nullptr;
+        const int rc = launch_gemm(gm, ix->dtype, kind, EPI_FILTER, p.main_grid, s);
         if (rc != CCR_OK) return rc;
         done = bounds[ph];
     }
@@ -450,6 +470,8 @@
     st.main_launches = 1 + (p.item_a ? 1 : 0) + (p.item_b ? 1 : 0);
     st.opt_rank = p.opt_rank;
     st.tile_cap = p.opt_rank ? p.tile_cap : 0;
+    st.main_grid = p.narrow ? 0 : p.main_grid;
+    st.side_cus = p.side_cus;
     st.skipped_tiles = p.skip_sampled ? p.sample_tiles : 0;
     st.main_tile_queries = p.narrow ? 0 : p.tile_q;
     st.n_candidates = (int64_t)ncand;
@@ -647,11 +669,13 @@
     ix->id_out = id_out;
     const bool async = (flags & CCR_SEARCH_ASYNC) != 0;
     const int plan_flags = flags & ~CCR_SEARCH_ASYNC;
-    if (!(ix->plan_nq == n_q && ix->plan_k == k && ix->plan_flags == plan_flags)) {
-        ix->plan = make_plan(ix->n_rows, ix->dim, n_q, k, plan_flags, ix->num_cu, ix->knobs);
+    const bool side_hint = side_hint_take(ix->device);
+    if (!(ix->plan_nq == n_q && ix->plan_k == k && ix->plan_flags == plan_flags && ix->plan_side_hint == side_hint)) {
+        ix->plan = make_plan(ix->n_rows, ix->dim, n_q, k, plan_flags, ix->num_cu, ix->knobs, side_hint);
         ix->plan_nq = n_q;
         ix->plan_k = k;
         ix->plan_flags = plan_flags;
+        ix->plan_side_hint = side_hint;
     }
     const Plan p = ix->plan;
     if (!workspace || ws_bytes < p.total || (uintptr_t)workspace % 256 != 0) {
@@ -659,6 +683,7 @@
         return CCR_ERR_WORKSPACE;
     }
     const SearchWs w = search_ws(p, ix->n_rows, ix->dim, n_q, k, (char *)workspace);
+    ix->side_arrive = w.arrive;
 
     if (!ix->have_events) {
         for (int i = 0; i < EV_COUNT; ++i) CCR_HIP_CHECK(hipEventCreate(&ix->ev[i]));
diff --git a/crowd-coachable-recommendations_amd/csrc/ccr_common.h b/crowd-coachable-recommendations_amd/csrc/ccr_common.h
--- a/crowd-coachable-recommendations_amd/csrc/ccr_common.h
+++ b/crowd-coachable-recommendations_amd/csrc/ccr_common.h
@@ -124,6 +124,7 @@
     uint2 *cand;
     uint32_t *cnt;
     CandLayout lay;
+    uint32_t *arrive;
     float *gmax;
     float *store;
     int64_t store_pitch;
diff --git a/crowd-coachable-recommendations_amd/csrc/ccr_index.h b/crowd-coachable-recommendations_amd/csrc/ccr_index.h
--- a/crowd-coachable-recommendations_amd/csrc/ccr_index.h
+++ b/crowd-coachable-recommendations_amd/csrc/ccr_index.h
@@ -6,6 +6,7 @@
 
 enum MainKernel { MAIN_32X32, MAIN_16X16, MAIN_WIDE };
 int launch_gemm(const GemmArgs &a, int dt, MainKernel kind, int epi, int grid, hipStream_t s);
+int launch_main_pass_gate(const uint32_t *arrive, uint32_t want, hipStream_t s);
 int launch_shard_header(const ccr_shard_header &h, void *message, hipStream_t s);
 int ensure_dynamic_lds(const void *kernel, size_t lds);
 int launch_row_norms(const uint16_t *X, int dt, int64_t rows, int dim, float *norms, uint32_t *max_bits, uint32_t *tile_bits,
@@ -112,6 +113,8 @@
     volatile uint32_t *host_flags;
     ccr::Plan plan;
     int plan_nq, plan_k, plan_flags;
+    bool plan_side_hint;
+    const uint32_t *side_arrive;
     ccr_search_stats stats;
     struct {
         bool active;
diff --git a/crowd-coachable-recommendations_amd/csrc/ccr_main_pass.hip b/crowd-coachable-recommendations_amd/csrc/ccr_main_pass.hip
--- a/crowd-coachable-recommendations_amd/csrc/ccr_main_pass.hip
+++ b/crowd-coachable-recommendations_amd/csrc/ccr_main_pass.hip
@@ -47,6 +47,10 @@
         return main_item(i, xcd, a.qblocks, a.qgroups, a.qsplit, a.ranges, a.n_vt, r, qb);
     }
 };
+
+__device__ __forceinline__ void announce_arrival(const GemmArgs &a) {
+    if (a.arrive != nullptr && threadIdx.x == 0) atomicAdd(a.arrive, 1u);
+}
 
 
 template <int ET>
@@ -235,6 +239,7 @@
     const int schunk = (lane & 3) ^ S::src_swizzle(srow);
     const S mfma(lane, wd, wq);
 
+    if constexpr (EPI == EPI_FILTER) announce_arrival(a);
     const ItemWalk walk(a);
     for (int item = walk.first(a); item < walk.end; item += walk.step) {
         int r, qb;
@@ -473,6 +478,7 @@
         lane_lds = (uint32_t)((ln & 15) * 64 + (((ln >> 4) ^ (((ln >> 2) & 1) << 1)) << 4));
     }
 
+    announce_arrival(a);
     const ItemWalk walk(a);
     for (int item = walk.first(a); item < walk.end; item += walk.step) {
         int r, qb;
@@ -739,6 +745,23 @@
     return launch_kernel(k, RING * (size_t)SUB_BYTES, a, grid, s);
 }
 
+constexpr int GATE_MAX_POLLS = 1024;
+constexpr long long GATE_MAX_TICKS = 30000;
+__global__ __launch_bounds__(64) void main_pass_gate_kernel(const uint32_t *arrive, uint32_t want) {
+    const long long t0 = wall_clock64();
+    for (int i = 0; i < GATE_MAX_POLLS; ++i) {
+        if (__hip_atomic_load(arrive, __ATOMIC_RELAXED, __HIP_MEMORY_SCOPE_AGENT) >= want) return;
+        if (wall_clock64() - t0 > GATE_MAX_TICKS) return;
+        __builtin_amdgcn_s_sleep(64);
+    }
+}
+
+int launch_main_pass_gate(const uint32_t *arrive, uint32_t want, hipStream_t s) {
+    hipLaunchKernelGGL(main_pass_gate_kernel, dim3(1), dim3(64), 0, s, arrive, want);
+    CCR_LAUNCH_CHECK();
+    return CCR_OK;
+}
+
 int launch_gemm(const GemmArgs &a, int dt, MainKernel kind, int epi, int grid, hipStream_t s) {
     return dispatch_half(dt, [&](auto et) { return launch_gemm_of<decltype(et)::value>(a, kind, epi, grid, s); });
 }
diff --git a/crowd-coachable-recommendations_amd/csrc/ccr_plan.h b/crowd-coachable-recommendations_amd/csrc/ccr_plan.h
--- a/crowd-coachable-recommendations_amd/csrc/ccr_plan.h
+++ b/crowd-coachable-recommendations_amd/csrc/ccr_plan.h
@@ -23,6 +23,7 @@
     int thr_phases;
     int narrow_groups;
     int tile_cap;
+    int side_cus;
 };
 struct KnobDef {
     const char *env;
@@ -36,7 +37,7 @@
     {"CCR_NARROW", &Knobs::narrow, -1},            {"CCR_NARROW_GRID", &Knobs::narrow_grid, 0},   {"CCR_SKIP_SAMPLED", &Knobs::skip_sampled, -1},
     {"CCR_SKIP_LIST", &Knobs::skip_list, 1},       {"CCR_QSPLIT", &Knobs::qsplit, -1},            {"CCR_WIDE", &Knobs::wide, -1},
     {"CCR_THR_PHASES", &Knobs::thr_phases, 0},     {"CCR_NARROW_GROUPS", &Knobs::narrow_groups, NARROW_MAX_GROUPS},
-    {"CCR_TILE_CAP", &Knobs::tile_cap, 0},
+    {"CCR_TILE_CAP", &Knobs::tile_cap, 0},         {"CCR_SIDE_CUS", &Knobs::side_cus, -1},
 };
 static_assert(sizeof(KNOB_DEFS) / sizeof(KNOB_DEFS[0]) * sizeof(int) == sizeof(Knobs), "a row for every knob");
 inline Knobs default_knobs() {
@@ -70,6 +71,8 @@
     int cap;
     CandLayout cand;
     int grid;
+    int main_grid;
+    int side_cus;
     int rescore_cap;
     int rescore_regular;
     int select_compact;
@@ -91,7 +94,10 @@
 
 constexpr int FALLBACK_ROWS = 16;
 
-Plan make_plan(int64_t n_rows, int dim, int n_q, int k, int flags, int num_cu, const Knobs &kn);
+Plan make_plan(int64_t n_rows, int dim, int n_q, int k, int flags, int num_cu, const Knobs &kn, bool side_hint = false);
+constexpr int SIDE_CUS_MAX_DIV = 4;
+double side_main_pass_ms(const Plan &p, int dim);
+double side_pack_ms(int64_t n_rows, int dim);
 
 inline int64_t round_up(int64_t v, int64_t m) { return (v + m - 1) / m * m; }
 int pick_qgroups(int qblocks, int dim, const Knobs &kn, int tile_q = TILE_Q);
@@ -107,6 +113,7 @@
     uint32_t *cnt;
     uint2 *cand;
     uint32_t *flag_count, *flag_list;
+    uint32_t *arrive;
     unsigned long long *stat_cand;
     uint32_t *top;
     float *thr_safe, *cq_safe, *dense;
diff --git a/crowd-coachable-recommendations_amd/csrc/ccr_plan.hip b/crowd-coachable-recommendations_amd/csrc/ccr_plan.hip
--- a/crowd-coachable-recommendations_amd/csrc/ccr_plan.hip
+++ b/crowd-coachable-recommendations_amd/csrc/ccr_plan.hip
@@ -127,10 +127,10 @@
 
 static void range_window(const Plan &p, const Knobs &kn, int64_t &r_hi, int64_t &target) {
     int64_t max_lists = p.rescore_cap > 512 ? 2048 : 1024;
-    if ((max_lists / p.sublists) * p.main_qblocks < p.grid) max_lists = 2048;
+    if ((max_lists / p.sublists) * p.main_qblocks < p.main_grid) max_lists = 2048;
     if (kn.max_lists >= 64 && kn.max_lists < max_lists) max_lists = kn.max_lists;
     r_hi = std::min<int64_t>(max_lists / p.sublists, round_up(std::max<int64_t>(1, p.tiles / 8), NUM_XCD));
-    target = std::min<int64_t>(r_hi, round_up(std::max<int64_t>(NUM_XCD, (int64_t)p.grid * 6 / p.main_qblocks), NUM_XCD));
+    target = std::min<int64_t>(r_hi, round_up(std::max<int64_t>(NUM_XCD, (int64_t)p.main_grid * 6 / p.main_qblocks), NUM_XCD));
 }
 
 static double sample_cost(const Plan &p, int64_t smp) {
@@ -146,7 +146,7 @@
 };
 
 static void price_range_count(const Plan &p, int k, const Knobs &kn, int64_t smp, int64_t R, int64_t target, bool reprice_skipped, Best &best) {
-    const int nrc = NUM_XCD / p.main_qgroups, qb_per = p.main_qblocks / p.main_qgroups, per_x = p.grid / NUM_XCD;
+    const int nrc = NUM_XCD / p.main_qgroups, qb_per = p.main_qblocks / p.main_qgroups, per_x = p.main_grid / NUM_XCD;
     const double qscale = query_scale(p);
     const double select_per_range = 0.1 * qscale, hit_w = 0.014 * qscale, phase_w = 3.0;
     const double fs = (double)smp / (double)p.tiles;
@@ -170,7 +170,7 @@
             best.offer(opt, {smp, R, 0, 0, rank, skip ? 1 : 0});
         }
     }
-    if (reprice_skipped || kn.progressive == 0 || p.narrow || !(items > per_x && (double)p.tiles / (double)R >= 8.0)) return;
+    if (reprice_skipped || kn.progressive == 0 || p.narrow || p.side_cus || !(items > per_x && (double)p.tiles / (double)R >= 8.0)) return;
     const double fa = (double)per_x / (double)items;
     best.offer((1.0 + rounds(items - per_x)) * item_cost + phase_w + hit_w * survivors(fa, 0.0) + common, {smp, R, per_x, 0, 0, 0});
     if (kn.max_phases < 3) return;
@@ -199,6 +199,7 @@
     int64_t n_rows;
     int dim, n_q, k, flags, num_cu;
     const Knobs &kn;
+    int side_cus;
 };
 
 static int64_t sample_for(const Plan &p, int k, int64_t div) {
@@ -219,6 +220,8 @@
     p.tiles = (s.n_rows + TILE_DOCS - 1) / TILE_DOCS;
     p.full_tiles = s.n_rows / TILE_DOCS;
     p.grid = std::max(NUM_XCD, s.num_cu / NUM_XCD * NUM_XCD);
+    p.side_cus = std::min(s.side_cus, p.grid - NUM_XCD);
+    p.main_grid = p.grid - p.side_cus;
     p.mfma16 = mfma16;
     p.sublists = p.mfma16 ? 8 : 4;
     p.rescore_cap = p.rescore_regular = std::min(8192, std::max(256, 2 * pow2_ceil(s.k)));
@@ -309,7 +312,7 @@
     const int k = s.k;
     const double join_rows = 256.0 * (double)p.sample_tiles * (1.0 - pow(1.0 - std::min(1.0, (double)k / (double)s.n_rows), 16.0));
     const double need = (double)k + (double)(k / 4) + 1.5 * join_rows + TILE_DOCS + 16;
-    const double saved = 0.5 * (double)p.sample_tiles * p.main_qblocks * tile_cost(p) / (double)p.grid;
+    const double saved = 0.5 * (double)p.sample_tiles * p.main_qblocks * tile_cost(p) / (double)p.main_grid;
     const bool pays = 0.065 * join_rows * query_scale(p) < saved;
     if (need > 8192.0 || (s.kn.skip_sampled < 0 && !pays)) {
         p.skip_sampled = 0;
@@ -401,7 +404,7 @@
     return rows;
 }
 
-static Plan make_plan_for(const Search &s, int mfma16) {
+static Plan plan_once(const Search &s, int mfma16) {
     Plan p = plan_geometry(s, mfma16);
     const int64_t sample = decide_fused(s, p);
     if (p.fused) {
@@ -421,6 +424,13 @@
     return p;
 }
 
+static Plan make_plan_for(const Search &s, int mfma16) {
+    Plan p = plan_once(s, mfma16);
+    if (s.side_cus == 0 || (p.fused && !p.narrow && p.item_a == 0 && p.item_b == 0)) return p;
+    const Search whole = {s.n_rows, s.dim, s.n_q, s.k, s.flags, s.num_cu, s.kn, 0};
+    return plan_once(whole, mfma16);
+}
+
 SearchWs search_ws(const Plan &p, int64_t n_rows, int dim, int n_q, int k, char *base) {
     SearchWs w;
     memset(&w, 0, sizeof(w));
@@ -429,7 +439,8 @@
     auto take = [&](size_t bytes) { return at(b.take(bytes)); };
     if (!p.fused) {
         w.flag_count = (uint32_t *)take(64 + (size_t)n_q * 4);
-        w.flag_list = w.flag_count + 16;
+        w.arrive = w.flag_count + 4;
+    w.flag_list = w.flag_count + 16;
         w.dense_bytes = (size_t)p.dense_rows_per_chunk * (n_rows + 3) * 4;
         w.dense = (float *)take(w.dense_bytes);
         w.total = b.off;
@@ -444,6 +455,7 @@
     w.cand = (uint2 *)take((size_t)p.cand_recs * 8);
     w.flag_count = (uint32_t *)take(64 + (size_t)n_q * 4);
     w.stat_cand = (unsigned long long *)(w.flag_count + 2);
+    w.arrive = w.flag_count + 4;
     w.flag_list = w.flag_count + 16;
     w.cand_bytes = (char *)w.flag_count - (char *)w.cand;
     w.top = (uint32_t *)take(p.item_b ? (nq_pad + (size_t)n_q * k) * 4 : 0);
@@ -467,13 +479,55 @@
     return w;
 }
 
-Plan make_plan(int64_t n_rows, int dim, int n_q, int k, int flags, int num_cu, const Knobs &kn) {
-    const Search s = {n_rows, dim, n_q, k, flags, num_cu, kn};
+static Plan plan_on_best_kernel(const Search &s) {
+    const Knobs &kn = s.kn;
     if (kn.mfma16 >= 0) return make_plan_for(s, kn.mfma16 ? 1 : 0);
-    if (k <= 512) return make_plan_for(s, 1);
+    if (s.k <= 512) return make_plan_for(s, 1);
     const Plan p32 = make_plan_for(s, 0);
     if (p32.fused && p32.ranges * 8 <= 2048) return make_plan_for(s, 1);
     return p32;
 }
 
-}
+constexpr double SIDE_TILE_MS = 0.0198, SIDE_PACK_CU_GBPS = 40.0, SIDE_PACK_ALL_GBPS = 5300.0, SIDE_SELECT_COVER_MS = 0.35;
+
+static double main_pass_units(const Plan &p) {
+    const int nrc = NUM_XCD / p.main_qgroups, qb_per = p.main_qblocks / p.main_qgroups, per_x = p.main_grid / NUM_XCD;
+    const int64_t items = p.ranges / nrc * qb_per, walked = p.tiles - (p.skip_sampled ? p.sample_tiles : 0);
+    return (double)((items + per_x - 1) / per_x) * ((double)((walked + p.ranges - 1) / p.ranges) + 0.15) * tile_cost(p);
+}
+static double side_ms_per_unit(const Search &s) { return SIDE_TILE_MS * (double)s.dim / 768.0; }
+static double side_pack_bytes(const Search &s) { return (double)s.n_rows * s.dim * 6.0; }
+double side_main_pass_ms(const Plan &p, int dim) { return main_pass_units(p) * SIDE_TILE_MS * (double)dim / 768.0; }
+double side_pack_ms(int64_t n_rows, int dim) { return (double)n_rows * dim * 6.0 / (SIDE_PACK_ALL_GBPS * 1e6); }
+
+static int side_cus_for(const Search &s, const Plan &whole) {
+    const Knobs &kn = s.kn;
+    if (kn.side_cus == 0 || !whole.fused || whole.narrow || whole.item_a || whole.item_b) return 0;
+    if (kn.side_cus > 0) return (int)std::min<int64_t>(round_up(kn.side_cus, NUM_XCD), whole.grid - NUM_XCD);
+    const double main_ms = main_pass_units(whole) * side_ms_per_unit(s), bytes = side_pack_bytes(s);
+    if (main_ms < side_pack_ms(s.n_rows, s.dim)) return 0;
+    const int want = (int)(bytes / (main_ms * SIDE_PACK_CU_GBPS * 1e6) / NUM_XCD + 0.5) * NUM_XCD;
+    return std::min(want, whole.grid / SIDE_CUS_MAX_DIV / NUM_XCD * NUM_XCD);
+}
+
+static bool side_cus_pay(const Search &s, const Plan &whole, const Plan &carved) {
+    const double unit = side_ms_per_unit(s), main_ms = main_pass_units(carved) * unit;
+    const double cost = main_ms - main_pass_units(whole) * unit;
+    const double pack_ms = side_pack_bytes(s) / (SIDE_PACK_ALL_GBPS * 1e6);
+    const double hidden = std::min(pack_ms, main_ms * carved.side_cus * SIDE_PACK_CU_GBPS / SIDE_PACK_ALL_GBPS);
+    const double pass = carved.opt_rank ? estimated_pass(carved.opt_rank, sample_fraction(carved), s.k) : conservative_pass(carved, s.k);
+    const double select_ms = (0.1 * carved.ranges + 0.014 * pass) * query_scale(carved) * unit;
+    return cost + std::min(select_ms, SIDE_SELECT_COVER_MS) < hidden;
+}
+
+Plan make_plan(int64_t n_rows, int dim, int n_q, int k, int flags, int num_cu, const Knobs &kn, bool side_hint) {
+    Search s = {n_rows, dim, n_q, k, flags, num_cu, kn, 0};
+    const Plan whole = plan_on_best_kernel(s);
+    s.side_cus = side_hint ? side_cus_for(s, whole) : 0;
+    if (s.side_cus == 0) return whole;
+    const Plan carved = plan_on_best_kernel(s);
+    if (carved.side_cus == 0 || (kn.side_cus < 0 && !side_cus_pay(s, whole, carved))) return whole;
+    return carved;
+}
+
+}
diff --git a/include/ccr_retrieval.h b/include/ccr_retrieval.h
--- a/include/ccr_retrieval.h
+++ b/include/ccr_retrieval.h
@@ -49,6 +49,8 @@
     int32_t main_tile_queries;
     int32_t skipped_tiles;
     int32_t tile_cap;
+    int32_t main_grid;
+    int32_t side_cus;
 } ccr_search_stats;
 
 const char *ccr_last_error(void);
```

Result: faster. 274,900, median of 6 (+2.3%).
